# Hansard-T/FHE-Linformer

Measured on AMD Instinct MI355X. Metric: encrypted Linformer-d128 forward ms/sample, lower is better.
Workload: dtype u64

## Files before the change

### fhe-linformer_amd/csrc/context.cpp

```cpp
#include "context.h"
#include <hip/hip_runtime.h>
#include <algorithm>
#include <cstdio>
#include <cstdlib>
#include <cstring>
#include <sys/random.h>
#include <time.h>
#include <cxxabi.h>
#include <dlfcn.h>
#include <execinfo.h>

namespace fhelin {

template <class T>
const T* Context::upload_table(const std::vector<T>& v) {
    void* p = nullptr;
    size_t bytes = std::max<size_t>(v.size() * sizeof(T), 16);
    hip_check(hipMalloc(&p, bytes), "hipMalloc(table)");
    if (!v.empty()) hip_check(hipMemcpy(p, v.data(), v.size() * sizeof(T), hipMemcpyHostToDevice), "hipMemcpy(table)");
    table_allocs.push_back(p);
    return static_cast<const T*>(p);
}
template const u64* Context::upload_table<u64>(const std::vector<u64>&);
template const int* Context::upload_table<int>(const std::vector<int>&);
template const u32* Context::upload_table<u32>(const std::vector<u32>&);
template const double* Context::upload_table<double>(const std::vector<double>&);

static u64 mont_r(u64 m) { return (u64)((((u128)1) << 64) % m); }

static u64 prod_mod(const std::vector<u64>& ms, int skip, u64 t) {
    u64 r = 1 % t;
    for (int i = 0; i < (int)ms.size(); ++i)
        if (i != skip) r = h_mulmod(r, ms[i] % t, t);
    return r;
}

static void resolve_seed(Params& p) {
    if (p.have_seed_bytes) return;
    if (p.seed != 0) {
        std::memset(p.seed_bytes, 0, sizeof p.seed_bytes);
        for (int i = 0; i < 8; ++i) p.seed_bytes[i] = (uint8_t)(p.seed >> (8 * i));
    } else {
        size_t got = 0;
        while (got < sizeof p.seed_bytes) {
            const ssize_t n = getrandom(p.seed_bytes + got, sizeof p.seed_bytes - got, 0);
            if (n <= 0) throw Error(FHELIN_ERR_INTERNAL, "getrandom failed: no entropy for key generation");
            got += (size_t)n;
        }
    }
    p.have_seed_bytes = true;
}

static Params resolve_params(Params p) {
    resolve_seed(p);
    if (p.n_p < 0 && p.n_q >= 1 && p.dnum >= 1 && p.special_bits >= 1) {
        const int a = (p.n_q + p.dnum - 1) / p.dnum;
        const int first = p.first_bits + (std::min(a, p.n_q) - 1) * p.scale_bits;
        const int other = p.n_q > a ? std::min(a, p.n_q - a) * p.scale_bits : 0;
        p.n_p = (std::max(first, other) + p.special_bits - 1) / p.special_bits;
    }
    return p;
}

Context::Context(const Params& p_in) : prm(resolve_params(p_in)) {
    const Params& p = prm;
    if (p.log_n < 12 || p.log_n > 17) throw Error(FHELIN_ERR_ARG, "log_n must be in [12,17]");
    if (p.n_q < 1 || p.n_q > 64 || p.n_p < 0 || p.n_p > 16) throw Error(FHELIN_ERR_ARG, "bad limb counts");
    if (p.dnum < 1) throw Error(FHELIN_ERR_ARG, "dnum must be >= 1");
    if (p.first_bits > 60 || p.scale_bits > 60 || p.special_bits > 60) throw Error(FHELIN_ERR_ARG, "primes must be <= 60 bits");
    if (p.first_bits < 20 || p.scale_bits < 20 || (p.n_p > 0 && p.special_bits < 20)) throw Error(FHELIN_ERR_ARG, "primes must be >= 20 bits");
    if (p.log_slots < 1 || p.log_slots > p.log_n - 1) throw Error(FHELIN_ERR_ARG, "log_slots out of range");
    N = 1 << p.log_n;
    L = p.n_q - 1;
    K = p.n_p;
    alpha = (p.n_q + p.dnum - 1) / p.dnum;
    if (alpha > 16) throw Error(FHELIN_ERR_ARG, "digit size > 16 limbs not supported");
    if ((p.n_q + alpha - 1) / alpha > 16) throw Error(FHELIN_ERR_ARG, "more than 16 key-switching digits not supported");
    try {
        chain = make_prime_chain(p.log_n, p.n_q, p.first_bits, p.scale_bits, p.n_p, p.special_bits);
    } catch (const std::exception& e) {
        throw Error(FHELIN_ERR_ARG, std::string("prime chain: ") + e.what());
    }
    moduli = chain.q;
    moduli.insert(moduli.end(), chain.p.begin(), chain.p.end());
    for (u64 q : moduli)
        if (q >> 60) throw Error(FHELIN_ERR_ARG, "prime chain: a modulus is >= 2^60 (lower scale_bits or first_bits)");
    for (u64 q : moduli) {
        barrett.push_back(h_barrett(q));
        tw.push_back(make_twiddles(q, p.log_n));
    }
    sf_real.assign(p.n_q + 1, 0.0L);
    sf_real[0] = (long double)chain.q[L];
    for (int k = 0; k < L; ++k) sf_real[k + 1] = sf_real[k] * sf_real[k] / (long double)chain.q[L - k];

    pool.fill_word = DevicePool::parse_fill(std::getenv("FHELIN_POOL_FILL"));

    if (p.device < 0) return;

    int ndev = 0;
    if (hipGetDeviceCount(&ndev) != hipSuccess || ndev <= 0)
        throw Error(FHELIN_ERR_NO_DEVICE, "no HIP device visible: the fhe-linformer_amd engine has no CPU fallback");
    if (p.device >= ndev) throw Error(FHELIN_ERR_ARG, "device index out of range");
    hip_check(hipSetDevice(p.device), "hipSetDevice");
    hip_check(hipStreamCreateWithFlags(&stream, hipStreamNonBlocking), "hipStreamCreate");
    main_stream = stream;
    own_stream = true;
    {
        int want = 2;
        if (const char* e = std::getenv("FHELIN_LANES")) want = std::atoi(e);
        n_lanes = std::max(0, std::min(want, DevicePool::MAX_LANES - 1));
        for (int k = 1; k <= n_lanes; ++k) {
            hip_check(hipStreamCreateWithFlags(&lane_stream[k], hipStreamNonBlocking), "hipStreamCreate(lane)");
            hip_check(hipEventCreateWithFlags(&lane_event[k], hipEventDisableTiming), "hipEventCreate(lane)");
        }
        hip_check(hipEventCreateWithFlags(&fork_event, hipEventDisableTiming), "hipEventCreate(fork)");
        pool.lane_stream[0] = main_stream;
        for (int k = 1; k <= n_lanes; ++k) pool.lane_stream[k] = lane_stream[k];
        pool.have_streams = true;
        if (const char* e = std::getenv("FHELIN_ASYNC")) async_lanes = std::atoi(e) != 0;
        if (const char* e = std::getenv("FHELIN_FUSE_MODDOWN")) fuse_moddown = std::atoi(e) != 0;
        if (const char* e = std::getenv("FHELIN_FUSE_FINISH")) fuse_finish = std::atoi(e) != 0;
        if (const char* e = std::getenv("FHELIN_HOST_ENCODE")) host_encode = std::atoi(e) != 0;
        if (const char* e = std::getenv("FHELIN_DEVICE_DECODE")) device_decode = std::atoi(e) != 0;
        if (const char* e = std::getenv("FHELIN_ROT_GATHER")) rot_gather = std::atoi(e) != 0;
        if (const char* e = std::getenv("FHELIN_FUSE_LIFT")) fuse_lift = std::atoi(e) != 0;
        if (const char* e = std::getenv("FHELIN_LDS_DIGITS")) lds_digits = std::atoi(e) != 0;
        if (const char* e = std::getenv("FHELIN_FUSE_ACCP_ROWS")) fuse_accp_rows = std::atoi(e);
        if (const char* e = std::getenv("FHELIN_ACCP_ROWS_MIN_VECS")) accp_rows_min_vecs = std::atoi(e);
        if (const char* e = std::getenv("FHELIN_FUSE_ACCQ_ROWS")) fuse_accq_rows = std::atoi(e);
        if (const char* e = std::getenv("FHELIN_ACCQ_ROWS_MIN_VECS")) accq_rows_min_vecs = std::atoi(e);
        if (const char* e = std::getenv("FHELIN_NTT_TRACE")) trace_small_ntt = std::atoi(e);
        if (const char* e = std::getenv("FHELIN_SCALAR_TRACE")) trace_scalar = std::atoi(e);
        if (const char* e = std::getenv("FHELIN_HOST_WAITS")) trace_waits = std::atoi(e) != 0;
    }
    hip_check(hipEventCreate(&ev_start), "hipEventCreate");
    stage_words = (size_t)2 << p.log_n;
    for (int i = 0; i < STAGE_SLOTS; ++i) {
        hip_check(hipHostMalloc(reinterpret_cast<void**>(&stage_buf[i]), stage_words * sizeof(u64), hipHostMallocDefault), "hipHostMalloc(stage)");
        hip_check(hipEventCreateWithFlags(&stage_ev[i], hipEventDisableTiming), "hipEventCreate(stage)");
    }
    hip_check(hipHostMalloc(reinterpret_cast<void**>(&small_buf), (size_t)SMALL_SLOTS * SMALL_WORDS * sizeof(u64), hipHostMallocDefault), "hipHostMalloc(stage, small)");
    for (int i = 0; i < SMALL_SLOTS; ++i) hip_check(hipEventCreateWithFlags(&small_ev[i], hipEventDisableTiming), "hipEventCreate(stage, small)");
    hip_check(hipEventCreate(&ev_stop), "hipEventCreate");
    has_device = true;

    const int nl = (int)moduli.size();
    {
        std::vector<u64> bar(2 * nl), ninv(8 * nl, 0);
        for (int i = 0; i < nl; ++i) {
            bar[2 * i] = barrett[i].r0;
            bar[2 * i + 1] = barrett[i].r1;
            ninv[8 * i] = tw[i].n_inv;
            ninv[8 * i + 1] = tw[i].n_inv_s;
            ninv[8 * i + 2] = tw[i].w1_n_inv;
            ninv[8 * i + 3] = tw[i].w1_n_inv_s;
            int bits = 0;
            while (bits < 64 && (moduli[i] >> bits)) ++bits;
            if (bits >= 12 && bits <= 60) {
                ninv[8 * i + 4] = (u64)(bits - 10);
                ninv[8 * i + 5] = (u64)((((u128)1) << (bits + 22)) / moduli[i]);
            }
        }
        dt.log_n = p.log_n;
        dt.n_limbs = nl;
        dt.moduli = upload_table(moduli);
        dt.barrett = upload_table(bar);
        {
            std::vector<u64> qi(nl);
            for (int i = 0; i < nl; ++i) {
                u64 x = moduli[i];
                for (int it = 0; it < 6; ++it) x *= 2 - moduli[i] * x;
                qi[i] = x;
            }
            dt.qinv = upload_table(qi);
            std::vector<u64> mr(2 * (size_t)nl);
            for (int i = 0; i < nl; ++i) {
                mr[2 * i] = mont_r(moduli[i]);
                mr[2 * i + 1] = h_shoup(mr[2 * i], moduli[i]);
            }
            dt.mont = upload_table(mr);
        }
        dt.ninv = upload_table(ninv);
        std::vector<u64> f((size_t)nl * 2 * N), g((size_t)nl * 2 * N);
        for (int i = 0; i < nl; ++i) {
            std::memcpy(&f[(size_t)i * 2 * N], tw[i].fwd.data(), sizeof(u64) * 2 * N);
            std::memcpy(&g[(size_t)i * 2 * N], tw[i].inv.data(), sizeof(u64) * 2 * N);
        }
        dt.tw_fwd = upload_table(f);
        dt.tw_inv = upload_table(g);
        const size_t tiles = N >> 12;
        const size_t per_limb = tiles * 15 * 256 * 2;
        for (int dir = 0; dir < 2; ++dir) {
            const std::vector<u64>& src = dir ? g : f;
            std::vector<u64> r((size_t)nl * per_limb);
            for (int i = 0; i < nl; ++i)
                for (size_t T = 0; T < tiles; ++T)
                    for (int kb = 0; kb < 4; ++kb)
                        for (int j = 0; j < (8 >> kb); ++j)
                            for (size_t tau = 0; tau < 256; ++tau) {
                                const size_t idx = (N >> (kb + 1)) + ((((T << 8) | tau)) << (3 - kb)) + j;
                                const size_t s_ = (size_t)(8 >> kb) - 1 + j;
                                const size_t o = (size_t)i * per_limb + ((T * 15 + s_) * 256 + tau) * 2;
                                r[o] = src[(size_t)i * 2 * N + 2 * idx];
                                r[o + 1] = src[(size_t)i * 2 * N + 2 * idx + 1];
                            }
            (dir ? dt.tw_rows_inv : dt.tw_rows_fwd) = upload_table(r);
        }
    }
    {
        std::vector<u64> phatinv(2 * std::max(K, 1)), phatmod((size_t)std::max(K, 1) * (L + 1)), pinv(2 * (L + 1));
        for (int j = 0; j < K; ++j) {
            u64 pj = chain.p[j];
            u64 hat = prod_mod(chain.p, j, pj);
            u64 inv = h_invmod(hat, pj);
            phatinv[2 * j] = inv;
            phatinv[2 * j + 1] = h_shoup(inv, pj);
            for (int t = 0; t <= L; ++t) phatmod[(size_t)j * (L + 1) + t] = pack30(h_mulmod(prod_mod(chain.p, j, chain.q[t]), mont_r(chain.q[t]), chain.q[t]));
        }
        for (int t = 0; t <= L; ++t) {
            u64 qt = chain.q[t];
            u64 pm = prod_mod(chain.p, -1, qt);
            u64 inv = K > 0 ? h_invmod(pm, qt) : 1;
            pinv[2 * t] = inv;
            pinv[2 * t + 1] = h_shoup(inv, qt);
        }
        d_phatinv = upload_table(phatinv);
        d_phatmod = upload_table(phatmod);
        d_pinv = upload_table(pinv);
        std::vector<u64> pmod(2 * (L + 1));
        for (int t = 0; t <= L; ++t) {
            pmod[2 * t] = prod_mod(chain.p, -1, chain.q[t]);
            pmod[2 * t + 1] = h_shoup(pmod[2 * t], chain.q[t]);
        }
        d_pmod = upload_table(pmod);
        std::vector<u64> qlinv((size_t)(L + 1) * (L + 1) * 2, 0), qlmod((size_t)(L + 1) * (L + 1), 0);
        for (int l = 0; l <= L; ++l)
            for (int t = 0; t < l; ++t) {
                u64 qt = chain.q[t];
                u64 r = chain.q[l] % qt;
                u64 inv = h_invmod(r, qt);
                qlmod[(size_t)l * (L + 1) + t] = r;
                qlinv[((size_t)l * (L + 1) + t) * 2] = inv;
                qlinv[((size_t)l * (L + 1) + t) * 2 + 1] = h_shoup(inv, qt);
            }
        d_qlinv = upload_table(qlinv);
        d_qlmod = upload_table(qlmod);
    }
    lvl.resize(L + 2);
    for (int ell = 1; ell <= L + 1; ++ell) {
        LevelTables& lt = lvl[ell];
        lt.ell = ell;
        lt.beta = digits_at(ell);
        const int nt = ell + K;
        std::vector<u64> hatinv(2 * ell), hatmod((size_t)ell * nt, 0), hatmod2((size_t)ell * nt, 0);
        std::vector<int> tab((size_t)lt.beta * nt, -1);
        for (int j = 0; j < lt.beta; ++j) {
            const int lo = j * alpha, hi = std::min((j + 1) * alpha, ell);
            std::vector<u64> dig(chain.q.begin() + lo, chain.q.begin() + hi);
            for (int i = lo; i < hi; ++i) {
                u64 qi = chain.q[i];
                u64 inv = h_invmod(prod_mod(dig, i - lo, qi), qi);
                hatinv[2 * i] = inv;
                hatinv[2 * i + 1] = h_shoup(inv, qi);
                for (int t = 0; t < nt; ++t) {
                    u64 mt = t < ell ? chain.q[t] : chain.p[t - ell];
                    const u64 hr = h_mulmod(prod_mod(dig, i - lo, mt), mont_r(mt), mt);
                    hatmod[(size_t)i * nt + t] = pack30(hr);
                    hatmod2[(size_t)i * nt + t] = pack30(h_mulmod(hr, mont_r(mt), mt));
                }
            }
            for (int t = 0; t < nt; ++t) {
                bool own = t >= lo && t < hi;
                tab[(size_t)j * nt + t] = own ? -1 : (t < ell ? limb_id_q(t) : limb_id_p(t - ell));
            }
        }
        lt.up_hatinv = upload_table(hatinv);
        lt.up_hatmod = upload_table(hatmod);
        lt.up_hatmod_r2 = upload_table(hatmod2);
        lt.ext_limb_tab = upload_table(tab);
        std::vector<int> ktab(nt);
        for (int t = 0; t < nt; ++t) ktab[t] = t < ell ? limb_id_q(t) : limb_id_p(t - ell);
        lt.key_limb_tab = upload_table(ktab);
        if (ell >= 2 && K >= 1) {
// ... 240 lines not shown
```

### fhe-linformer_amd/csrc/context.h

```cpp
#pragma once
#include <cstdint>
#include <map>
#include <memory>
#include <stdexcept>
#include <string>
#include <unordered_map>
#include <vector>
#include <hip/hip_runtime_api.h>
#include "../../include/fhelin.h"
#include "hostmath.h"
#include "pool.h"
#include "kernels_elem.h"

namespace fhelin {

struct Params {
    int log_n = 16;
    int n_q = 24;
    int first_bits = 55;
    int scale_bits = 52;
    int n_p = 6;
    int special_bits = 60;
    int dnum = 4;
    int log_slots = 14;
    int hamming = 192;
    uint64_t seed = 0;
    uint8_t seed_bytes[32] = {};
    bool have_seed_bytes = false;
    int device = 0;
};

struct LevelTables {
    int ell = 0;
    int beta = 0;
    const u64* up_hatinv = nullptr;
    const u64* up_hatmod = nullptr;
    const u64* up_hatmod_r2 = nullptr;
    const int* ext_limb_tab = nullptr;
    const int* key_limb_tab = nullptr;
    const u64* md_hatinv = nullptr;
    const u64* md_hatmod = nullptr;
    const u64* md_minv = nullptr;
    const u64* md_mmod = nullptr;
    const int* mdx_limb_tab = nullptr;
};

struct OpStats {
    u64 limb_ntt = 0;
    u64 keyswitch = 0;
    u64 keyswitch_limbs = 0;
    u64 rescale = 0;
    u64 ct_pt_mult = 0;
    u64 bootstrap = 0;
    u64 encode = 0;
    u64 rescale_limbs = 0;
    u64 ct_pt_limbs = 0;
};

struct Context {
    Params prm;
    OpStats stats;
    int N = 0;
    int L = 0;
    int K = 0;
    int alpha = 0;
    PrimeChain chain;
    std::vector<u64> moduli;
    std::vector<Barrett> barrett;
    std::vector<TwiddleTable> tw;
    std::vector<long double> sf_real;

    bool has_device = false;
    hipStream_t stream = nullptr;
    hipStream_t main_stream = nullptr;
    bool own_stream = false;
    int n_lanes = 0;
    hipStream_t lane_stream[DevicePool::MAX_LANES] = {};
    hipEvent_t lane_event[DevicePool::MAX_LANES] = {};
    hipEvent_t fork_event = nullptr;
    bool async_lanes = true;
    int async_rr = 0;
    u64 lane_seq[DevicePool::MAX_LANES] = {};
    std::vector<std::pair<u64, std::shared_ptr<void>>> lane_hold[DevicePool::MAX_LANES];
    void release_holds(int lane, u64 up_to_seq);
    void fork_lanes();
    void join_lanes();
    DevicePool pool;
    hipStream_t stream_of(int lane) const { return pool.lane_stream[lane]; }
    void select_lane(int lane) {
        stream = stream_of(lane);
        pool.cur_lane = lane;
    }
    void set_main_stream(hipStream_t s) {
        stream = main_stream = pool.lane_stream[0] = s;
        own_stream = false;
    }
    struct LaneScope {
        Context& c;
        hipStream_t was_stream;
        int was_lane;
        LaneScope(Context& ctx, int k) : c(ctx), was_stream(ctx.stream), was_lane(ctx.pool.cur_lane) { c.select_lane(k); }
        ~LaneScope() {
            c.stream = was_stream;
            c.pool.cur_lane = was_lane;
        }
    };
    DeviceTables dt{};
    std::vector<void*> table_allocs;
    hipEvent_t ev_start = nullptr, ev_stop = nullptr;

    static constexpr int STAGE_SLOTS = 64;
    u64* stage_buf[STAGE_SLOTS] = {};
    hipEvent_t stage_ev[STAGE_SLOTS] = {};
    bool stage_used[STAGE_SLOTS] = {};
    int stage_next = 0;
    size_t stage_words = 0;
    static constexpr int SMALL_SLOTS = 256;
    static constexpr size_t SMALL_WORDS = 8192;
    u64* small_buf = nullptr;
    hipEvent_t small_ev[SMALL_SLOTS] = {};
    bool small_used[SMALL_SLOTS] = {};
    int small_next = 0;
    void upload_async(u64* dst, const u64* src, size_t words);

    const u64* d_phatinv = nullptr;
    const u64* d_phatmod = nullptr;
    const u64* d_pinv = nullptr;
    const u64* d_pmod = nullptr;
    const u64* d_qlinv = nullptr;
    const u64* d_qlmod = nullptr;
    std::vector<LevelTables> lvl;
    std::map<u64, const u32*> automorph_maps;

    explicit Context(const Params& p);
    ~Context();
    Context(const Context&) = delete;
    Context& operator=(const Context&) = delete;

    void require_device() const;
    template <class T> T* dalloc(size_t count) { return static_cast<T*>(pool.alloc(count * sizeof(T))); }
    template <class T> Scratch<T> scratch(size_t count) { return Scratch<T>(pool, count); }
    template <class T> const T* upload_table(const std::vector<T>& v);
    int limb_id_q(int i) const { return i; }
    int limb_id_p(int j) const { return L + 1 + j; }
    int digits_at(int ell) const { return (ell + alpha - 1) / alpha; }
    u64 galois_element(long rot_index) const;
    int stride = 1;
    bool stride_explicit = false;
    bool stride_locked = false;
    u64 rot_element(int rot_index) const { return stride == 1 ? galois_element(rot_index) : galois_element((long)stride * rot_index); }
    struct PhysicalScope {
        Context& c;
        int was;
        explicit PhysicalScope(Context& ctx) : c(ctx), was(ctx.stride) { c.stride = 1; }
        ~PhysicalScope() { c.stride = was; }
    };
    const u32* automorph_map(u64 galois);
    const u32* automorph_inverse_of(const u32* map);
    std::map<const u32*, const u32*> automorph_inverse;
    u32 automorph_ginv_of(const u32* map) const;
    std::map<const u32*, u32> automorph_ginv;
    bool fuse_finish = true;
    bool fuse_moddown = false;
    bool host_encode = false;
    bool device_decode = false;
    bool rot_gather = true;
    bool fuse_lift = true;
    int fuse_accp_rows = 1;
    int accp_rows_min_vecs = 0;
    int fuse_accq_rows = 1;
    int accq_rows_min_vecs = 0;
    bool lds_digits = true;
    struct FftDev {
        const u32* rot = nullptr;
        const double* ksi = nullptr;
    };
    std::map<int, FftDev> fft_dev;
    void sync();
    void ntt(const LimbBatch& b, bool inverse, int active = -1) {
        stats.limb_ntt += (u64)(active >= 0 ? active : b.nvec);
        if (trace_small_ntt && b.nvec <= trace_small_ntt) note_small_ntt(b.nvec);
        launch_ntt(dt, b, inverse, stream);
    }
    bool trace_waits = false;
    std::map<std::string, std::pair<u64, u64>> wait_sites;
    void note_wait(const char* site, u64 ns) {
        auto& e = wait_sites[site];
        e.first += 1;
        e.second += ns;
    }
    int trace_small_ntt = 0;
    std::map<std::string, std::pair<u64, u64>> small_ntt_sites;
    void note_small_ntt(int nvec);
    int trace_scalar = 0;
    std::map<std::string, std::pair<u64, u64>> scalar_sites;
    void note_scalar(int nvec);
    void ntt_epilogue(const LimbBatch& b, const NttEpilogue& ep) {
        stats.limb_ntt += (u64)b.nvec;
        if (trace_small_ntt && b.nvec <= trace_small_ntt) note_small_ntt(b.nvec);
        launch_ntt_epilogue(dt, b, ep, stream);
    }
    void ntt_epilogue_product(const LimbBatch& b, const NttEpilogue& ep, const NttProduct& p) {
        stats.limb_ntt += (u64)b.nvec;
        if (trace_small_ntt && b.nvec <= trace_small_ntt) note_small_ntt(b.nvec);
        launch_ntt_epilogue_product(dt, b, ep, p, stream);
    }
};

}
```

### fhe-linformer_amd/csrc/evaluator.cpp

```cpp
#include "evaluator.h"
#include <map>
#include <set>
#include <hip/hip_runtime.h>
#include <cmath>
#include <cstring>

namespace fhelin {

DevBlock::~DevBlock() {
    if (d && ctx) {
        try { ctx->pool.free(d); } catch (...) {}
    }
}
Ciphertext::~Ciphertext() {
    if (async_ev) (void)hipEventDestroy(async_ev);
    if (d && ctx && !block) {
        try { ctx->pool.free(d); } catch (...) {}
    }
}
Encoding::~Encoding() {
    if (ready) (void)hipEventDestroy(ready);
    if (d && ctx) {
        try { ctx->pool.free(d, lanes_ordered); } catch (...) {}
    }
}
EvalKey::~EvalKey() {
    if (d && ctx) {
        try { ctx->pool.free(d); } catch (...) {}
    }
    if (d_perm && ctx) {
        try { ctx->pool.free(d_perm); } catch (...) {}
    }
}

static void launch_ok(const char* what) { hip_check(hipGetLastError(), what); }

namespace {
template <class SameShape, class Emit>
void for_runs(size_t n, SameShape same, Emit emit) {
    size_t lo = 0;
    while (lo < n) {
        size_t hi = lo + 1;
        while (hi < n && hi - lo < (size_t)EwItems::MAX_ITEMS && same(lo, hi)) ++hi;
        emit(lo, hi);
        lo = hi;
    }
}

template <class Same, class Run>
std::vector<CtPtr> for_groups(size_t n, int limit, Same same, Run run) {
    std::vector<CtPtr> out(n);
    std::vector<char> done(n, 0);
    for (size_t first = 0; first < n; ++first) {
        if (done[first]) continue;
        std::vector<size_t> idx{first};
        for (size_t i = first + 1; i < n && (int)idx.size() < limit; ++i)
            if (!done[i] && same(first, i)) idx.push_back(i);
        std::vector<CtPtr> o = run(idx);
        for (size_t k = 0; k < idx.size(); ++k) {
            out[idx[k]] = std::move(o[k]);
            done[idx[k]] = 1;
        }
    }
    return out;
}

std::vector<CtPtr> pick(const std::vector<CtPtr>& v, const std::vector<size_t>& idx) {
    std::vector<CtPtr> o;
    o.reserve(idx.size());
    for (size_t i : idx) o.push_back(v[i]);
    return o;
}
}

CtPtr Evaluator::new_ct(int npoly, int ell, int deg, long double scale, int slots) {
    c_.require_device();
    if (ell < 1 || ell > c_.L + 1 || npoly < 1 || npoly > 3) throw Error(FHELIN_ERR_ARG, "new_ct: bad shape");
    auto ct = std::make_shared<Ciphertext>();
    ct->ctx = &c_;
    ct->npoly = npoly;
    ct->ell = ell;
    ct->deg = deg;
    ct->scale = scale;
    ct->slots = slots;
    ct->d = c_.dalloc<u64>(ct->words());
    c_.stride_locked = true;
    return ct;
}

CtPtr Evaluator::clone(const CtPtr& a) {
    CtPtr o = new_ct(a->npoly, a->ell, a->deg, a->scale, a->slots);
    hip_check(hipMemcpyAsync(o->d, a->d, a->words() * 8, hipMemcpyDeviceToDevice, c_.stream), "clone");
    return o;
}

std::vector<CtPtr> Evaluator::new_ct_batch(int count, int npoly, int ell, int deg, long double scale, int slots) {
    c_.require_device();
    if (count < 1 || ell < 1 || ell > c_.L + 1 + (c_.K > 0 ? 1 : 0) || npoly < 1 || npoly > 3) throw Error(FHELIN_ERR_ARG, "new_ct_batch: bad shape");
    auto blk = std::make_shared<DevBlock>();
    blk->ctx = &c_;
    const size_t words = (size_t)npoly * ell * c_.N;
    blk->d = c_.dalloc<u64>(words * count);
    c_.stride_locked = true;
    std::vector<CtPtr> v;
    for (int i = 0; i < count; ++i) {
        auto ct = std::make_shared<Ciphertext>();
        ct->ctx = &c_;
        ct->npoly = npoly;
        ct->ell = ell;
        ct->deg = deg;
        ct->scale = scale;
        ct->slots = slots;
        ct->block = blk;
        ct->d = blk->d + words * i;
        v.push_back(ct);
    }
    return v;
}

u64* Evaluator::contiguous_base(const std::vector<CtPtr>& v) {
    if (v.empty() || !v[0]->block) return nullptr;
    const size_t words = v[0]->words();
    for (size_t i = 0; i < v.size(); ++i)
        if (v[i]->block != v[0]->block || v[i]->d != v[0]->d + words * i || v[i]->words() != words) return nullptr;
    return v[0]->d;
}

std::vector<CtPtr> Evaluator::make_contiguous(const std::vector<CtPtr>& v, int site) {
    if (v.size() <= 1 || contiguous_base(v)) return v;
    if (site >= 0 && site < 8) gather_copies[site] += v.size();
    std::vector<CtPtr> o = new_ct_batch((int)v.size(), v[0]->npoly, v[0]->ell, v[0]->deg, v[0]->scale, v[0]->slots);
    for (size_t lo = 0; lo < v.size(); lo += EwItems::MAX_ITEMS) {
        EwItems it;
        it.n = (int)std::min<size_t>(EwItems::MAX_ITEMS, v.size() - lo);
        it.vecs = v[0]->npoly * v[0]->ell;
        it.b_vecs = 0;
        for (int i = 0; i < it.n; ++i) {
            if (v[lo + i]->words() != v[0]->words()) throw Error(FHELIN_ERR_INTERNAL, "make_contiguous: operands of different shapes");
            it.out[i] = o[lo + i]->d;
            it.a[i] = v[lo + i]->d;
            it.b[i] = nullptr;
        }
        launch_ew_items(c_.dt, it, 4, v[0]->ell, c_.stream);
    }
    hip_check(hipGetLastError(), "batch gather");
    return o;
}

KeyPtr Evaluator::new_key(int max_ell) {
    c_.require_device();
    if (max_ell < 0 || max_ell > c_.L + 1) throw Error(FHELIN_ERR_ARG, "new_key: max_ell out of range");
    auto k = std::make_shared<EvalKey>();
    k->ctx = &c_;
    k->max_ell = max_ell ? max_ell : c_.L + 1;
    k->digits = c_.digits_at(k->max_ell);
    k->d = c_.dalloc<u64>(k->words());
    if (k->capped()) {
        hip_check(hipMemsetAsync(k->d, 0, k->words() * sizeof(u64), c_.stream), "hipMemsetAsync(capped key)");
    }
    c_.stride_locked = true;
    return k;
}

void Evaluator::bind_key(const EvalKey& key, int ell) {
    if (ell > key.max_ell) {
        std::string who = key.kind == 1 ? "relinearisation key" : key.kind == 3 ? "conjugation key" : "rotation key";
        if (key.kind != 1 && key.has_index) who += " for index " + std::to_string(key.index);
        if (key.kind != 1) who += " (Galois element " + std::to_string((unsigned long long)key.galois) + ")";
        throw Error(FHELIN_ERR_KEY, who + " is capped at " + std::to_string(key.max_ell) + " limbs: a key switch at " + std::to_string(ell) +
                                        " limbs was asked for");
    }
    if (usage_on) {
        int& m = usage[{key.kind, key.galois}];
        m = std::max(m, ell);
    }
}

void Evaluator::bind_rotations(const Rotations& rot, const std::vector<CtPtr>& v, bool rescales_first) {
    for (const CtPtr& x : v)
        for (int r = 0; r < rot.n; ++r) bind_key(*rot.key[r], rescales_first && x->deg >= 2 ? x->ell - 1 : x->ell);
}

void Evaluator::keyswitch(const u64* c_ntt, int ell, const EvalKey& key, u64* out, const u64* add0, const u64* add1,
                          const u32* map, const u64* post) {
    keyswitch_batch(1, c_ntt, 0, ell, key, out, 0, add0, add1, 0, map, post, 0);
}

void Evaluator::keyswitch_batch(int B, const u64* c_ntt, size_t c_stride, int ell, const EvalKey& key, u64* out, size_t out_stride,
                                const u64* add0, const u64* add1, size_t add_stride, const u32* map, const u64* post,
                                size_t post_stride) {
    keyswitch_impl(B, nullptr, c_ntt, c_stride, ell, &key, out, out_stride, add0, add1, add_stride, map, post, post_stride);
}

void Evaluator::keyswitch_rows(const KsRows& rows, const u64* c_ntt, size_t c_stride, int ell, u64* out, size_t out_stride,
                               const u64* add0, size_t add_stride) {
    const int B = (int)rows.keys.size();
    if (B < 1) return;
    if (B > KsShape::MAX_ROWS || rows.maps.size() != rows.keys.size()) throw Error(FHELIN_ERR_ARG, "keyswitch_rows: bad row count");
    keyswitch_impl(B, &rows, c_ntt, c_stride, ell, nullptr, out, out_stride, add0, nullptr, add_stride, nullptr, nullptr, 0);
}

void Evaluator::keyswitch_impl(int B, const KsRows* rows, const u64* c_ntt, size_t c_stride, int ell, const EvalKey* key, u64* out,
                               size_t out_stride, const u64* add0, const u64* add1, size_t add_stride, const u32* map, const u64* post,
                               size_t post_stride) {
    c_.require_device();
    if (c_.K < 1) throw Error(FHELIN_ERR_STATE, "hybrid key switching needs at least one special prime");
    if (B < 1) return;
    if (key) bind_key(*key, ell);
    else
        for (int b = 0; b < B; ++b) bind_key(*rows->keys[b], ell);
    KsShape sh = ks_shape(ell, B, {c_stride, out_stride, add_stride, post_stride});
    const bool shared = rows && rows->shared_input;
    if (rows) {
        sh.per_row = 1;
        sh.shared_input = shared ? 1 : 0;
        for (int b = 0; b < B; ++b) {
            sh.evk_row[b] = rows->keys[b]->d;
            sh.map_row[b] = rows->maps[b];
        }
    }
    KsShape shu = sh;
    shu.batch = shared ? 1 : B;
    c_.stats.keyswitch += (u64)B;
    c_.stats.keyswitch_limbs += (u64)B * ell;
    const bool identity = !map && !rows;
    const bool gather = !identity && !add1 && rot_in_gather();
    const u64* evk = key ? key->d : nullptr;
    if (gather) evk = set_gather(sh, rows ? rows->keys.data() : &key, rows ? rows->maps.data() : &map, add0, add_stride);
    Scratch<u64> ext = modup(shu, c_ntt, !gather);
    KsAcc acc = inner_product(sh, ext, evk, c_ntt, moddown_tail(gather ? KsOutput::Gathered : identity ? KsOutput::Identity : KsOutput::Scattered));
    moddown(acc, gather ? KsOut{out, nullptr, nullptr, post} : KsOut{out, add0, add1, post, map});
    launch_ok("keyswitch");
}


KsShape Evaluator::ks_shape(int ell, int batch, const KsStrides& st) const {
    return KsShape{ell, c_.K, c_.alpha, c_.lvl[ell].beta, c_.L + 1, batch, st.c, st.out, st.add, st.post};
}

Evaluator::KsTail Evaluator::moddown_tail(KsOutput o) const {
    const bool rows = o == KsOutput::Gathered || (o == KsOutput::Identity && (c_.fuse_moddown || c_.fuse_finish)) ||
                      (o == KsOutput::Scattered && c_.fuse_moddown) || (o == KsOutput::MergedSum && c_.fuse_finish && c_.rot_gather);
    return rows ? KsTail::RowPass : KsTail::Finish;
}

const u64* Evaluator::set_gather(KsShape& sh, const EvalKey* const* keys, const u32* const* maps, const u64* c0, size_t c0_stride) {
    const u64* evk = nullptr;
    for (int b = 0; b < (sh.per_row ? (sh.row_mod ? sh.row_mod : sh.batch) : 1); ++b) bind_key(*keys[b], sh.ell);
    sh.gather = 1;
    if (sh.per_row) {
        for (int b = 0; b < (sh.row_mod ? sh.row_mod : sh.batch); ++b) {
            sh.evk_row[b] = permuted(*keys[b], maps[b]);
            sh.ginv_row[b] = c_.automorph_ginv_of(maps[b]);
        }
    } else {
        evk = permuted(*keys[0], maps[0]);
        sh.map_row[0] = maps[0];
        sh.ginv = c_.automorph_ginv_of(maps[0]);
    }
    if (c0) {
        sh.gsrc = c0;
        sh.gsrc_stride = c0_stride;
        sh.gsrc_pmod = c_.d_pmod;
    }
    return evk;
}

Scratch<u64> Evaluator::modup(const KsShape& up, const u64* src, bool times_r2, int group2, size_t group2_stride) {
    const size_t N = c_.N;
    const int n = up.batch, ell = up.ell, nt = ell + c_.K;
    const LevelTables& lt = c_.lvl[ell];
    Scratch<u64> cc = c_.scratch<u64>((size_t)n * ell * N);
    {
        LimbBatch ib{cc, n * ell, nullptr, 0, ell, src};
        if (n > 1 && up.c_stride != (size_t)ell * N) {
            ib.src_group = ell;
            ib.src_group_stride = up.c_stride;
        }
        if (group2 > 0) {
            ib.src_group2 = group2;
            ib.src_group2_stride = group2_stride;
        }
        c_.ntt(ib, true);
    }
    Scratch<u64> ext = c_.scratch<u64>((size_t)n * lt.beta * nt * N);
    launch_modup_conv(c_.dt, up, ext, cc, src, lt.up_hatinv, times_r2 ? lt.up_hatmod_r2 : lt.up_hatmod, c_.stream);
    LimbBatch eb{ext, n * lt.beta * nt, lt.ext_limb_tab, 0, 1};
    eb.tab_len = lt.beta * nt;
    eb.lazy_out = true;
    c_.ntt(eb, false, n * (lt.beta * nt - ell));
    return ext;
}

bool Evaluator::accp_in_rows(const KsShape& sh, KsTail tail) const {
    const int K = c_.K, nvec = sh.batch * 2 * K;
    const bool measured_faster = !sh.n_rot && sh.beta <= 8;
    const bool want = c_.fuse_accp_rows >= 2 || (c_.fuse_accp_rows == 1 && measured_faster);
    return tail != KsTail::EditsAccP && want && !sh.accp_limbs && sh.k == K && nvec >= c_.accp_rows_min_vecs;
}

bool Evaluator::accq_in_rows(const KsShape& sh, KsTail tail) const {
    const bool measured_faster = sh.beta <= 8 && sh.batch * 2 * sh.ell >= c_.accq_rows_min_vecs;
    const bool want = c_.fuse_accq_rows >= 2 || (c_.fuse_accq_rows == 1 && measured_faster);
    return tail == KsTail::RowPass && !sh.n_rot && want;
}

Evaluator::KsAcc Evaluator::accumulators(const KsShape& sh, KsTail tail) {
    const size_t pairs = (size_t)sh.batch * 2 * c_.N;
    return KsAcc{sh, tail, c_.scratch<u64>(pairs * sh.ell), c_.scratch<u64>(pairs * (sh.accp_limbs ? sh.accp_limbs : sh.k)), {}};
}

Evaluator::KsAcc Evaluator::inner_product(const KsShape& shape, const u64* ext, const u64* evk, const u64* c_ntt, KsTail tail) {
    const int K = c_.K, nvec = shape.batch * 2 * K;
    KsAcc acc{shape, tail, {}, {}, {}};
    KsShape& sh = acc.sh;
    sh.accp_rows = accp_in_rows(sh, tail) ? 1 : 0;
    sh.accq_rows = sh.accp_rows && accq_in_rows(sh, tail) ? 1 : 0;
    if (!sh.accq_rows) acc.accQ = c_.scratch<u64>((size_t)sh.batch * 2 * sh.ell * c_.N);
    acc.accP = c_.scratch<u64>((size_t)nvec * c_.N);
    if (sh.n_rot) launch_ks_inner_multi(c_.dt, sh, acc.accQ, acc.accP, ext, c_ntt, c_.stream);
    else if (!sh.accq_rows) launch_ks_inner(c_.dt, sh, acc.accQ, acc.accP, ext, evk, c_ntt, c_.stream);
    if (!sh.accp_rows) return acc;
    acc.qprod = NttProduct{sh, ext, evk, sh.n_rot ? 1 : 0, c_ntt};
    c_.stats.limb_ntt += (u64)nvec;
    launch_ntt_rows_product(c_.dt, LimbBatch{acc.accP, nvec, nullptr, c_.L + 1, K}, acc.qprod, c_.stream);
    return acc;
}

void Evaluator::accp_inverse(KsAcc& acc) {
    const LimbBatch b{acc.accP, acc.sh.batch * 2 * c_.K, nullptr, c_.L + 1, c_.K};
    if (acc.sh.accp_rows) launch_ntt_cols_inverse(c_.dt, b, c_.stream);
    else c_.ntt(b, true);
}

static void made_for(bool ok, const char* tail) {
    if (!ok) throw Error(FHELIN_ERR_INTERNAL, std::string(tail) + ": the accumulator was made for another tail");
}

Scratch<u64> Evaluator::moddown_conv(KsAcc& acc) {
    const KsShape& sh = acc.sh;
    made_for(acc.tail == KsTail::RowPass || acc.tail == KsTail::Finish, "moddown");
    if (acc.tail == KsTail::RowPass && sh.gsrc && !sh.gsrc_pmod) throw Error(FHELIN_ERR_INTERNAL, "moddown: the row pass cannot gather");
    accp_inverse(acc);
    Scratch<u64> conv = c_.scratch<u64>((size_t)sh.batch * 2 * sh.ell * c_.N);
    launch_moddown_conv(c_.dt, sh, conv, acc.accP, c_.d_phatinv, c_.d_phatmod, c_.stream);
    if (acc.tail != KsTail::RowPass) c_.ntt(LimbBatch{conv, sh.batch * 2 * sh.ell, nullptr, 0, sh.ell}, false);
    return conv;
}

void Evaluator::moddown(KsAcc& acc, const KsOut& o) {
    Scratch<u64> conv = moddown_conv(acc);
    if (acc.tail == KsTail::RowPass) moddown_rows(acc, conv, o);
    else launch_moddown_finish(c_.dt, acc.sh, o.out, acc.accQ, conv, c_.d_pinv, o.add0, o.add1, o.map, o.post, c_.stream);
}

void Evaluator::moddown_rows(const KsAcc& acc, u64* conv, const KsOut& o) {
    const KsShape& sh = acc.sh;
    const int B = sh.batch, ell = sh.ell;
    const LimbBatch cb{conv, B * 2 * ell, nullptr, 0, ell};
    NttEpilogue ep;
    ep.acc = acc.accQ;
    ep.acc_poly_stride = (size_t)ell * c_.N;
    ep.out = o.out;
    ep.out_stride = sh.out_stride;
    ep.w = c_.d_pinv;
    ep.ell = ell;
    ep.add0 = o.add0;
    ep.add1 = o.add1;
    ep.add_stride = sh.add_stride;
    ep.post = o.post;
    ep.post_stride = sh.post_stride;
    if (sh.gather) {
    } else if (sh.per_row) {
        ep.per_row = 1;
        for (int b = 0; b < B; ++b) ep.invmap_row[b] = c_.automorph_inverse_of(sh.map_row[b]);
    } else if (o.map) {
        ep.invmap = c_.automorph_inverse_of(o.map);
    }
    if (sh.accq_rows) c_.ntt_epilogue_product(cb, ep, acc.qprod);
    else c_.ntt_epilogue(cb, ep);
}

void Evaluator::moddown_rescale(KsAcc& acc, u64* out) {
    const KsShape& sh = acc.sh;
    const size_t N = c_.N;
    const int B = sh.batch, ell = sh.ell;
    const LevelTables& lt = c_.lvl[ell];
    made_for(acc.tail == KsTail::Rescale || acc.tail == KsTail::EditsAccP, "moddown_rescale");
    accp_inverse(acc);
    Scratch<u64> top = c_.scratch<u64>((size_t)B * 2 * N);
    {
        LimbBatch tb{top, B * 2, nullptr, ell - 1, 1, acc.accQ + (size_t)(ell - 1) * N};
        tb.src_group = 1;
        tb.src_group_stride = (size_t)ell * N;
        c_.ntt(tb, true);
    }
    Scratch<u64> conv = c_.scratch<u64>((size_t)B * 2 * (ell - 1) * N);
    launch_moddown_rescale_conv(c_.dt, sh, conv, acc.accP, top, lt.md_hatinv, lt.md_hatmod, lt.md_mmod, c_.stream);
    moddown_rescale_finish(acc, out, conv, lt.md_minv);
}

void Evaluator::moddown_rescale_exact(KsAcc& acc, u64* out, u32 f2) {
    const KsShape& sh = acc.sh;
    const int B = sh.batch, ell = sh.ell, K = c_.K;
    const LevelTables& lt = c_.lvl[ell];
    made_for(acc.tail == KsTail::Exact, "moddown_rescale_exact");
    {
        LimbBatch ib{acc.accP, B * 2 * (K + 1), lt.mdx_limb_tab, 0, 1};
        ib.tab_len = K + 1;
        c_.ntt(ib, true);
    }
    Scratch<u64> conv = c_.scratch<u64>((size_t)B * 2 * (ell - 1) * c_.N);
    launch_moddown_rescale_exact_conv(c_.dt, sh, f2, conv, acc.accP, c_.d_phatinv, c_.d_phatmod, c_.d_pinv, c_.d_pmod,
                                      c_.d_qlmod + (size_t)(ell - 1) * (c_.L + 1), c_.stream);
    moddown_rescale_finish(acc, out, conv, lt.md_minv);
}

void Evaluator::moddown_rescale_finish(const KsAcc& acc, u64* out, u64* conv, const u64* minv) {
    const KsShape& sh = acc.sh;
    const int e1 = sh.ell - 1;
    const LimbBatch cb{conv, sh.batch * 2 * e1, nullptr, 0, e1};
    if (c_.fuse_finish) {
        NttEpilogue ep;
        ep.acc = acc.accQ;
        ep.acc_poly_stride = (size_t)sh.ell * c_.N;
        ep.out = out;
        ep.out_stride = sh.out_stride;
        ep.w = minv;
        ep.ell = e1;
        c_.ntt_epilogue(cb, ep);
        return;
    }
    c_.ntt(cb, false);
    launch_moddown_rescale_finish(c_.dt, sh, out, acc.accQ, conv, minv, c_.stream);
}

Evaluator::Rotations Evaluator::rotations(const int* indices, int n) {
    Rotations rot;
    rot.n = n;
    for (int r = 0; r < n; ++r) {
        const RotKey k = rotation_key(indices[r]);
        rot.key[r] = k.key.get();
        rot.map[r] = k.map;
        if (k.g % (u64)(c_.N / 256) != 1) rot.tiles_in_place = false;
    }
    return rot;
}

void Evaluator::set_rotations(KsShape& sh, const Rotations& rot, bool shared_digits, const u64* const* keys) {
    for (int r = 0; r < rot.n; ++r) bind_key(*rot.key[r], sh.ell);
    sh.n_rot = rot.n;
    for (int r = 0; r < rot.n; ++r) {
        sh.map_rot[r] = rot.map[r];
        sh.evk_rot[r] = keys ? keys[r] : permuted(*rot.key[r], rot.map[r]);
    }
    if (shared_digits) sh.lds_digits = c_.lds_digits && rot.tiles_in_place ? 1 : 0;
}

void Evaluator::rotation_sum(KsShape& sh, const u64* ext, const u64* base, size_t c0_stride, const KsOut& o) {
    const KsTail tail = moddown_tail(KsOutput::MergedSum);
    sh.gsrc = base;
    sh.gsrc_stride = c0_stride;
    if (tail == KsTail::RowPass) sh.gsrc_pmod = c_.d_pmod;
    KsAcc acc = inner_product(sh, ext, nullptr, base + (size_t)sh.ell * c_.N, tail);
    moddown(acc, o);
}

Scratch<u64> Evaluator::debug_ks_accp(const u64* ext, int ell, int batch, const int* indices, int n_rot) {
    const size_t pn = (size_t)ell * c_.N;
    if (ell < 1 || ell > c_.L + 1 || batch < 1 || n_rot < 0 || n_rot > (int)KsShape::MAX_ROT) throw Error(FHELIN_ERR_ARG, "debug_ks_accp: bad shape");
    if (!n_rot && !relin_key) throw Error(FHELIN_ERR_KEY, "debug_ks_accp: no relinearisation key");
    if (!n_rot) bind_key(*relin_key, ell);
    KsShape sh = ks_shape(ell, batch, {pn});
    Scratch<u64> own = c_.scratch<u64>((size_t)batch * pn);
    hip_check(hipMemsetAsync(own, 0, (size_t)batch * pn * sizeof(u64), c_.stream), "hipMemsetAsync(debug_ks_accp)");
    if (n_rot) set_rotations(sh, rotations(indices, n_rot), true, nullptr);
    KsAcc acc = inner_product(sh, ext, n_rot ? nullptr : relin_key->d, own, KsTail::Finish);
    accp_inverse(acc);
    launch_ok("debug_ks_accp");
    return std::move(acc.accP);
}

void Evaluator::debug_ks_accq(const u64* ext, const u64* own, u64* conv, int ell, int batch, int index, u64* out) {
    const size_t pn = (size_t)ell * c_.N;
    if (ell < 1 || ell > c_.L + 1 || batch < 1) throw Error(FHELIN_ERR_ARG, "debug_ks_accq: bad shape");
    if (!index && !relin_key) throw Error(FHELIN_ERR_KEY, "debug_ks_accq: no relinearisation key");
    if (!index) bind_key(*relin_key, ell);
    KsShape sh = ks_shape(ell, batch, {pn, 2 * pn});
    const u64* evk = index ? nullptr : relin_key->d;
    if (index) {
        const RotKey k = rotation_key(index);
        const EvalKey* key = k.key.get();
        evk = set_gather(sh, &key, &k.map);
    }
    KsAcc acc = inner_product(sh, ext, evk, own, KsTail::RowPass);
    moddown_rows(acc, conv, KsOut{out});
    launch_ok("debug_ks_accq");
}

int Evaluator::slot_count(int slots) const { return slots > 0 ? slots : (1 << c_.prm.log_slots); }

Evaluator::RotKey Evaluator::rotation_key(int index) {
    const u64 g = c_.rot_element(index);
    auto it = rot_keys.find(g);
    if (it == rot_keys.end()) throw Error(FHELIN_ERR_KEY, "no rotation key for index " + std::to_string(index) + " (EvalRotateKeyGen list)");
    return RotKey{it->second, c_.automorph_map(g), g};
}

bool Evaluator::have_rotation_keys(const std::vector<int>& indices, int slots) const {
    const int ns = slot_count(slots);
    for (int r : indices) {
        if (r % ns == 0) return false;
        if (!rot_keys.count(c_.rot_element(r))) return false;
    }
    return !indices.empty();
}

const u64* Evaluator::permuted(const EvalKey& key, const u32* map) {
    if (key.d_perm) return key.d_perm;
    const int nvec = key.digits * 2 * (c_.L + 1 + c_.K);
    key.d_perm = c_.dalloc<u64>(key.words());
    launch_automorph_pack30(c_.dt, key.d_perm, key.d, map, nvec, c_.stream);
    launch_ok("key permutation");
    hip_check(hipStreamSynchronize(c_.stream), "key permutation sync");
    return key.d_perm;
}

std::vector<CtPtr> Evaluator::rotate_sum_batch(const std::vector<CtPtr>& vin, const std::vector<int>& indices) {
    if (vin.empty()) return {};
    const int R = (int)indices.size();
    if (R < 1 || R > KsShape::MAX_ROT) throw Error(FHELIN_ERR_ARG, "rotate_sum_batch: 1..7 rotations");
    if (!have_rotation_keys(indices, vin[0]->slots)) throw Error(FHELIN_ERR_KEY, "rotate_sum_batch: missing rotation key");
    if (c_.K < 1) throw Error(FHELIN_ERR_STATE, "hybrid key switching needs at least one special prime");
    const Rotations rot = rotations(indices.data(), R);
    bind_rotations(rot, vin);
    const size_t N = c_.N;
    return for_groups(vin.size(), batch_limit, [&](size_t f, size_t i) { return same_shape(*vin[f], *vin[i]); },
                      [&](const std::vector<size_t>& idx) {
        if (vin[idx[0]]->npoly != 2) throw Error(FHELIN_ERR_STATE, "rotate: ciphertext must have 2 components");
        const std::vector<CtPtr> chunk = make_contiguous(pick(vin, idx), 0);
        const int B = (int)chunk.size(), ell = chunk[0]->ell;
        const size_t pn = (size_t)ell * N, ctw = 2 * pn;
        std::vector<CtPtr> o = new_ct_batch(B, 2, ell, chunk[0]->deg, chunk[0]->scale, chunk[0]->slots);
        const u64* base = chunk[0]->d;
        KsShape sh = ks_shape(ell, B, {ctw, ctw, pn, ctw});
        set_rotations(sh, rot, true);
        int steps = 0;
        while ((1 << steps) < R + 1) ++steps;
        c_.stats.keyswitch += (u64)B * steps;
        c_.stats.keyswitch_limbs += (u64)B * steps * ell;
        {
            Scratch<u64> ext = modup(sh, base + pn, false);
            rotation_sum(sh, ext, base, ctw, KsOut{o[0]->d, nullptr, nullptr, base});
            launch_ok("rotate_sum_batch");
        }
        for (int b = 0; b < B; ++b) o[b]->scale = vin[idx[b]]->scale;
        return o;
    });
}

Evaluator::FoldedKey Evaluator::folded_key(const PtPtr& p, int index, long double scale) {
    const RotKey rk = rotation_key(index);
    for (size_t i = 0; i < folded_keys.size(); ++i) {
        const FoldedKey& f = folded_keys[i];
        if (f.pt.get() == p.get() && f.key.get() == rk.key.get() && f.index == index && f.scale == scale) {
            FoldedKey hit = f;
            if (i + 1 != folded_keys.size()) {
                folded_keys.erase(folded_keys.begin() + i);
                folded_keys.push_back(hit);
            }
            return hit;
        }
    }
    FoldedKey f;
    f.pt = p;
    f.key = rk.key;
    f.index = index;
    f.scale = scale;
    const int nl = c_.L + 1 + c_.K;
    f.enc = p->at(nl, scale);
    f.d = std::make_shared<DevBlock>();
    f.d->ctx = &c_;
    f.d->d = c_.dalloc<u64>(f.key->words());
    launch_fold_key(c_.dt, f.d->d, f.key->d, rk.map, f.enc->d, f.key->digits * 2 * nl, c_.stream);
    launch_ok("fold_key");
// ... 1010 lines not shown
}

void Evaluator::rescale_degree2(std::vector<CtPtr>& a, std::vector<CtPtr>* b, const char* two_components) {
    std::vector<CtPtr> need;
    std::map<const Ciphertext*, size_t> slot;
    for (const auto* side : {&a, b})
        for (size_t i = 0; side && i < side->size(); ++i) {
            const CtPtr& c = (*side)[i];
            if (two_components && c->npoly != 2) throw Error(FHELIN_ERR_STATE, two_components);
            if (c->deg >= 2 && !slot.count(c.get())) {
                slot[c.get()] = need.size();
                need.push_back(c);
            }
        }
    if (need.empty()) return;
    const std::vector<CtPtr> r = rescale_batch(need);
    for (auto* side : {&a, b})
        for (size_t i = 0; side && i < side->size(); ++i) {
            CtPtr& c = (*side)[i];
            if (c->deg >= 2) c = r[slot[c.get()]];
        }
}

std::vector<CtPtr> Evaluator::tensor_products(const std::vector<CtPtr>& x, const std::vector<CtPtr>& y, const std::vector<size_t>& idx) {
    const int B = (int)idx.size(), ell = x[idx[0]]->ell;
    std::vector<CtPtr> d = new_ct_batch(B, 3, ell, 2, 0, x[idx[0]]->slots);
    for (int k0 = 0; k0 < B; k0 += EwItems::MAX_ITEMS) {
        EwItems it;
        it.n = std::min(B - k0, (int)EwItems::MAX_ITEMS);
        for (int k = 0; k < it.n; ++k) {
            it.out[k] = d[k0 + k]->d;
            it.a[k] = x[idx[k0 + k]]->d;
            it.b[k] = y[idx[k0 + k]]->d;
        }
        launch_tensor_items(c_.dt, it, ell, c_.stream);
    }
    return d;
}

void Evaluator::product_operands(const std::vector<CtPtr>& a, const std::vector<CtPtr>& b, std::vector<CtPtr>& x, std::vector<CtPtr>& y) {
    std::vector<CtPtr> ra = a, rb = b;
    rescale_degree2(ra, &rb, "mult: operands must have 2 components");
    match_batch(ra, rb, x, y);
}

std::vector<CtPtr> Evaluator::mult_batch(const std::vector<CtPtr>& a, const std::vector<CtPtr>& b) {
    if (a.size() != b.size()) throw Error(FHELIN_ERR_ARG, "mult_batch: operand count mismatch");
    if (!relin_key) throw Error(FHELIN_ERR_KEY, "no relinearisation key (EvalMultKeyGen not called)");
    std::vector<CtPtr> x, y;
    product_operands(a, b, x, y);
    for (const CtPtr& xi : x) bind_key(*relin_key, xi->ell);
    std::vector<CtPtr> out = for_groups(a.size(), batch_limit, [&](size_t f, size_t i) { return x[i]->ell == x[f]->ell; },
                                        [&](const std::vector<size_t>& idx) {
        const int B = (int)idx.size(), ell = x[idx[0]]->ell;
        const size_t pn = (size_t)ell * c_.N;
        const std::vector<CtPtr> d = tensor_products(x, y, idx);
        std::vector<CtPtr> o = new_ct_batch(B, 2, ell, 2, 0, x[idx[0]]->slots);
        keyswitch_batch(B, d[0]->d + 2 * pn, 3 * pn, ell, *relin_key, o[0]->d, 2 * pn, d[0]->d, d[0]->d + pn, 3 * pn, nullptr, nullptr, 0);
        for (int k = 0; k < B; ++k) {
            const size_t i = idx[k];
            o[k]->deg = x[i]->deg + y[i]->deg;
            o[k]->scale = x[i]->scale * y[i]->scale;
        }
        return o;
    });
    launch_ok("mult_batch");
    return out;
}

std::vector<CtPtr> Evaluator::mult_affine_rescale_batch(const std::vector<CtPtr>& a, const std::vector<CtPtr>& b, int f, double cadd,
                                                        const std::vector<CtPtr>& sub) {
    if (a.size() != b.size() || (!sub.empty() && sub.size() != a.size())) throw Error(FHELIN_ERR_ARG, "mult_affine_rescale_batch: operand count mismatch");
    if (f != 1 && f != 2) throw Error(FHELIN_ERR_ARG, "mult_affine_rescale_batch: factor 1 or 2");
    if (!relin_key) throw Error(FHELIN_ERR_KEY, "no relinearisation key (EvalMultKeyGen not called)");
    if (c_.K < 1 || c_.K + 1 > 16) throw Error(FHELIN_ERR_STATE, "mult_affine_rescale_batch: 1..15 special primes");
    std::vector<CtPtr> ra = a, rb = b, x(a.size()), y(a.size());
    rescale_degree2(ra, &rb, "mult: operands must have 2 components");
    for (size_t i = 0; i < a.size(); ++i) match(ra[i], rb[i], x[i], y[i]);
    for (const CtPtr& xi : x) bind_key(*relin_key, xi->ell);
    const size_t N = c_.N;
    const int K = c_.K, L1 = c_.L + 1;
    hipStream_t s = c_.stream;
    auto product_scale = [&](size_t i) { return x[i]->scale * y[i]->scale; };
    return for_groups(a.size(), batch_limit,
                      [&](size_t f0, size_t i) { return x[i]->ell == x[f0]->ell && fabsl(product_scale(i) / product_scale(f0) - 1.0L) < 1e-12L; },
                      [&](const std::vector<size_t>& idx) {
        const size_t first = idx[0];
        const int B = (int)idx.size(), ell = x[first]->ell;
        if (ell < 2) throw Error(FHELIN_ERR_STATE, "mult_affine_rescale_batch: no limb left to drop");
        const size_t pn = (size_t)ell * N;
        const long double sc = product_scale(first);
        const std::vector<CtPtr> d = tensor_products(x, y, idx);
        std::vector<CtPtr> sadj;
        if (!sub.empty()) {
            for (int k = 0; k < B; ++k) sadj.push_back(adjust(sub[idx[k]], ell, 2, sc));
            sadj = make_contiguous(sadj, 7);
        }
        ScalarSet cst;
        if (cadd != 0.0) real_to_scalars(c_, (long double)cadd * sc, ell, cst);
        KsShape sh = ks_shape(ell, B, {3 * pn, (size_t)2 * (ell - 1) * N, pn});
        c_.stats.keyswitch += (u64)B;
        c_.stats.keyswitch_limbs += (u64)B * ell;
        c_.stats.rescale += (u64)B;
        c_.stats.rescale_limbs += (u64)B * ell;
        const u64* c_ntt = d[0]->d + 2 * pn;
        std::vector<CtPtr> o = new_ct_batch(B, 2, ell - 1, 1, 0, x[first]->slots);
        {
            Scratch<u64> ext = modup(sh, c_ntt, true);
            KsAcc acc = inner_product(sh, ext, relin_key->d, c_ntt, f == 2 ? KsTail::EditsAccP : KsTail::Rescale);
            launch_affine_acc(c_.dt, sh, acc.accQ, d[0]->d, sadj.empty() ? nullptr : sadj[0]->d, cst, cadd != 0.0 ? 1 : 0, f, c_.d_pmod, s);
            if (f == 2) launch_ew_add(c_.dt, acc.accP, acc.accP, acc.accP, B * 2 * K, B * 2 * K, L1, K, s);
            moddown_rescale(acc, o[0]->d);
            launch_ok("mult_affine_rescale_batch");
        }
        for (int k = 0; k < B; ++k) o[k]->scale = product_scale(idx[k]) / (long double)c_.chain.q[ell - 1];
        return o;
    });
}

std::vector<CtPtr> Evaluator::mult_affine_unmerged(const std::vector<CtPtr>& a, const std::vector<CtPtr>& b, const std::vector<AffineSpec>& spec) {
    std::vector<CtPtr> t = mult_batch(a, b);
    const size_t n = t.size();
    {
        std::vector<size_t> pos;
        std::vector<CtPtr> sel;
        for (size_t i = 0; i < n; ++i)
            if (spec[i].f == 2) {
                pos.push_back(i);
                sel.push_back(t[i]);
            }
        if (!sel.empty()) {
            const std::vector<CtPtr> r = add_batch(sel, sel);
            for (size_t j = 0; j < pos.size(); ++j) t[pos[j]] = r[j];
        }
    }
    for (size_t i = 0; i < n; ++i)
        if (spec[i].cadd != 0.0) t[i] = add_real(t[i], spec[i].cadd);
    for (const bool neg : {true, false}) {
        std::vector<size_t> pos;
        std::vector<CtPtr> sel, ad;
        for (size_t i = 0; i < n; ++i)
            if (spec[i].addend && spec[i].negate == neg) {
                pos.push_back(i);
                sel.push_back(t[i]);
                ad.push_back(spec[i].addend);
            }
        if (sel.empty()) continue;
        const std::vector<CtPtr> r = neg ? sub_batch(sel, ad) : add_batch(sel, ad);
        for (size_t j = 0; j < pos.size(); ++j) t[pos[j]] = r[j];
    }
    return rescale_batch(t);
}

std::vector<CtPtr> Evaluator::mult_affine_batch(const std::vector<CtPtr>& a, const std::vector<CtPtr>& b, const std::vector<AffineSpec>& spec) {
    if (a.size() != b.size() || spec.size() != a.size()) throw Error(FHELIN_ERR_ARG, "mult_affine_batch: operand count mismatch");
    if (!relin_key) throw Error(FHELIN_ERR_KEY, "no relinearisation key (EvalMultKeyGen not called)");
    for (const AffineSpec& sp : spec) {
        if (sp.f != 1 && sp.f != 2) throw Error(FHELIN_ERR_ARG, "mult_affine_batch: factor 1 or 2");
        if (sp.addend && sp.addend->npoly != 2) throw Error(FHELIN_ERR_STATE, "add: component count mismatch");
    }
    if (!exact_products_on()) return mult_affine_unmerged(a, b, spec);
    const size_t n = a.size();
    std::vector<CtPtr> x, y;
    product_operands(a, b, x, y);
    for (const CtPtr& xi : x) bind_key(*relin_key, xi->ell);
    for (size_t i = 0; i < n; ++i)
        if (x[i]->ell < 2 || (spec[i].addend && spec[i].addend->ell < x[i]->ell)) return mult_affine_unmerged(x, y, spec);
    const size_t N = c_.N;
    const int K = c_.K;
    hipStream_t s = c_.stream;
    static_assert(AffineItems::MAX_ITEMS <= EwItems::MAX_ITEMS, "the tensor products of a group are one launch");
    return for_groups(n, std::min(batch_limit, (int)AffineItems::MAX_ITEMS), [&](size_t f, size_t i) { return x[i]->ell == x[f]->ell; },
                      [&](const std::vector<size_t>& idx) {
        const size_t first = idx[0];
        const int B = (int)idx.size(), ell = x[first]->ell;
        const size_t pn = (size_t)ell * N;
        const std::vector<CtPtr> d = tensor_products(x, y, idx);
        AffineItems items;
        std::vector<CtPtr> adj(B);
        std::map<std::pair<const Ciphertext*, long double>, CtPtr> adjusted;
        std::vector<u64> cst((size_t)B * ell, 0);
        for (int k = 0; k < B; ++k) {
            const size_t i = idx[k];
            const AffineSpec& sp = spec[i];
            const long double sc = x[i]->scale * y[i]->scale;
            if (sp.f == 2) items.f2 |= 1u << k;
            if (sp.addend) {
                const CtPtr& ad = sp.addend;
                const std::pair<const Ciphertext*, long double> key{ad.get(), sc};
                auto hit = ad->deg == 1 ? adjusted.find(key) : adjusted.end();
                if (hit != adjusted.end()) {
                    adj[k] = hit->second;
                } else {
                    adj[k] = ad->ell == ell && ad->deg == 2 ? ad : adjust(ad, ell, 2, sc);
                    if (ad->deg == 1) adjusted[key] = adj[k];
                }
                items.add[k] = adj[k]->d;
                if (sp.negate) items.neg |= 1u << k;
            }
            if (sp.cadd != 0.0) {
                ScalarSet one;
                real_to_scalars(c_, (long double)sp.cadd * sc, ell, one);
                for (int l = 0; l < ell; ++l) cst[(size_t)k * ell + l] = one.v[2 * l];
                items.cst |= 1u << k;
            }
        }
        Scratch<u64> dcst = c_.scratch<u64>(cst.size());
        if (items.cst) c_.upload_async(dcst, cst.data(), cst.size());
        KsShape sh = ks_shape(ell, B, {3 * pn, (size_t)2 * (ell - 1) * N, pn});
        sh.accp_limbs = K + 1;
        c_.stats.keyswitch += (u64)B;
        c_.stats.keyswitch_limbs += (u64)B * ell;
        c_.stats.rescale += (u64)B;
        c_.stats.rescale_limbs += (u64)B * ell;
        const u64* c_ntt = d[0]->d + 2 * pn;
        std::vector<CtPtr> o = new_ct_batch(B, 2, ell - 1, 1, 0, x[first]->slots);
        {
            Scratch<u64> ext = modup(sh, c_ntt, true);
            KsAcc acc = accumulators(sh, KsTail::Exact);
            launch_ks_inner(c_.dt, sh, acc.accQ, acc.accP, ext, relin_key->d, c_ntt, s);
            launch_affine_acc_items(c_.dt, sh, items, acc.accQ, acc.accP, d[0]->d, dcst, c_.d_pmod, s);
            moddown_rescale_exact(acc, o[0]->d, items.f2);
            launch_ok("mult_affine_batch");
        }
        for (int k = 0; k < B; ++k) o[k]->scale = x[idx[k]]->scale * y[idx[k]]->scale / (long double)c_.chain.q[ell - 1];
        return o;
    });
}

std::vector<CtPtr> Evaluator::add_plain_batch(const std::vector<CtPtr>& v, const PtPtr& p) {
    std::vector<CtPtr> out(v.size());
    for_runs(v.size(), [&](size_t a, size_t b) { return v[a]->npoly == v[b]->npoly && v[a]->ell == v[b]->ell; },
             [&](size_t lo, size_t hi) {
                 const CtPtr& f = v[lo];
                 std::vector<CtPtr> o = new_ct_batch((int)(hi - lo), f->npoly, f->ell, f->deg, f->scale, f->slots);
                 EwItems it;
                 it.n = (int)(hi - lo);
                 it.vecs = f->npoly * f->ell;
                 it.b_vecs = f->ell;
                 for (size_t i = lo; i < hi; ++i) {
                     auto enc = p->at(v[i]->ell, v[i]->scale);
                     o[i - lo]->deg = v[i]->deg;
                     o[i - lo]->scale = v[i]->scale;
                     it.out[i - lo] = o[i - lo]->d;
                     it.a[i - lo] = v[i]->d;
                     it.b[i - lo] = enc->d;
                     out[i] = o[i - lo];
                 }
                 launch_ew_items(c_.dt, it, 3, f->ell, c_.stream);
             });
    launch_ok("add_plain_batch");
    return out;
}

CtPtr Evaluator::rotate_add(const CtPtr& a, int index) {
    if (index % slot_count(a) == 0) return add(a, a);
    const RotKey k = rotation_key(index);
    return raw_rotate(a, k.g, *k.key, true, k.map);
}

CtPtr Evaluator::raw_mult_relin(const CtPtr& a, const CtPtr& b, const EvalKey& key) {
    if (a->npoly != 2 || b->npoly != 2 || a->ell != b->ell) throw Error(FHELIN_ERR_STATE, "mult: operands must be 2-component, same level");
    const int ell = a->ell;
    const size_t pn = (size_t)ell * c_.N;
    Scratch<u64> d = c_.scratch<u64>(3 * pn);
    launch_tensor(c_.dt, d, a->d, b->d, ell, c_.stream);
    CtPtr o = new_ct(2, ell, a->deg + b->deg, a->scale * b->scale, a->slots);
    keyswitch(d + 2 * pn, ell, key, o->d, d, d + pn, nullptr);
    return o;
}

CtPtr Evaluator::raw_modraise(const CtPtr& a, int new_ell) {
    if (a->ell != 1) throw Error(FHELIN_ERR_STATE, "modraise: the input must have exactly one limb (q0)");
    if (new_ell < 1 || new_ell > c_.L + 1) throw Error(FHELIN_ERR_ARG, "modraise: bad target limb count");
    const size_t N = c_.N;
    const int P = a->npoly;
    hipStream_t s = c_.stream;
    Scratch<u64> coef = c_.scratch<u64>((size_t)P * N);
    LimbBatch ib{coef, P, nullptr, 0, 1, a->d};
    c_.ntt(ib, true);
    CtPtr up = new_ct(P, new_ell, a->deg, a->scale, a->slots);
    launch_modraise(c_.dt, up->d, coef, P, 0, new_ell, s);
    c_.ntt(LimbBatch{up->d, P * new_ell, nullptr, 0, new_ell}, false);
    launch_ok("modraise");
    return up;
}

std::vector<CtPtr> Evaluator::raw_modraise_batch(const std::vector<CtPtr>& vin, int new_ell) {
    if (vin.size() <= 1) {
        std::vector<CtPtr> out;
        for (const CtPtr& a : vin) out.push_back(raw_modraise(a, new_ell));
        return out;
    }
    for (const CtPtr& a : vin)
        if (a->ell != 1 || a->npoly != vin[0]->npoly) throw Error(FHELIN_ERR_STATE, "modraise: the inputs must have exactly one limb (q0) and one shape");
    if (new_ell < 1 || new_ell > c_.L + 1) throw Error(FHELIN_ERR_ARG, "modraise: bad target limb count");
    std::vector<CtPtr> in = make_contiguous(vin, 7);
    const size_t N = c_.N;
    const int B = (int)in.size(), P = in[0]->npoly * B;
    hipStream_t s = c_.stream;
    Scratch<u64> coef = c_.scratch<u64>((size_t)P * N);
    c_.ntt(LimbBatch{coef, P, nullptr, 0, 1, in[0]->d}, true);
    std::vector<CtPtr> up = new_ct_batch(B, in[0]->npoly, new_ell, 1, 0, in[0]->slots);
    launch_modraise(c_.dt, up[0]->d, coef, P, 0, new_ell, s);
    c_.ntt(LimbBatch{up[0]->d, P * new_ell, nullptr, 0, new_ell}, false);
    launch_ok("modraise_batch");
    coef.reset();
    for (int b = 0; b < B; ++b) {
        up[b]->deg = vin[b]->deg;
        up[b]->scale = vin[b]->scale;
        up[b]->slots = vin[b]->slots;
    }
    return up;
}

CtPtr Evaluator::rescale(const CtPtr& a) {
    CtPtr o = raw_rescale(a);
    o->scale = a->scale / (long double)c_.chain.q[a->ell - 1];
    o->deg = a->deg > 1 ? a->deg - 1 : 1;
    return o;
}

CtPtr Evaluator::level_reduce(const CtPtr& a, int new_ell) {
    if (new_ell == a->ell) return a;
    if (new_ell < 1 || new_ell > a->ell) throw Error(FHELIN_ERR_ARG, "level_reduce: bad target");
    CtPtr o = new_ct(a->npoly, new_ell, a->deg, a->scale, a->slots);
    const size_t N = c_.N;
    hip_check(hipMemcpy2DAsync(o->d, (size_t)new_ell * N * 8, a->d, (size_t)a->ell * N * 8, (size_t)new_ell * N * 8, a->npoly,
                               hipMemcpyDeviceToDevice, c_.stream), "level_reduce");
    return o;
}

CtPtr Evaluator::mult_int(const CtPtr& a, u64 k, bool raise_deg, long double new_scale, int keep_ell) {
    const int ell = keep_ell > 0 ? std::min(keep_ell, a->ell) : a->ell;
    ScalarSet sc;
    for (int i = 0; i < ell; ++i) {
        u64 q = c_.chain.q[i];
        u64 v = k % q;
        sc.v[2 * i] = v;
        sc.v[2 * i + 1] = h_shoup(v, q);
    }
    CtPtr o = new_ct(a->npoly, ell, raise_deg ? a->deg + 1 : a->deg, new_scale, a->slots);
    if (c_.trace_scalar) c_.note_scalar(a->npoly * ell);
    launch_ew_scalar(c_.dt, o->d, a->d, sc, a->npoly * ell, 0, ell, c_.stream, ell < a->ell ? a->ell : 0);
    launch_ok("mult_int");
    return o;
}

std::vector<CtPtr> Evaluator::adjust_deg1_batch(const std::vector<CtPtr>& v, int ell, long double scale) {
    return adjust_deg1_batch(v, ell, std::vector<long double>(v.size(), scale));
}

std::vector<CtPtr> Evaluator::adjust_deg1_batch(const std::vector<CtPtr>& v, int ell, const std::vector<long double>& scales) {
    if (scales.size() != v.size()) throw Error(FHELIN_ERR_ARG, "adjust_deg1_batch: one target scale per ciphertext");
    std::vector<CtPtr> out(v.size()), pending, src;
    std::vector<size_t> pos;
    for (size_t i = 0; i < v.size(); ++i) {
        CtPtr cur = v[i];
        if (cur->ell < ell) throw Error(FHELIN_ERR_STATE, "adjust: cannot raise a ciphertext to a lower level");
        if (cur->deg == 2) cur = rescale(cur);
        if (cur->ell == ell) {
            out[i] = cur;
            continue;
        }
        src.push_back(cur);
        pos.push_back(i);
    }
    if (!src.empty()) {
        const long double qdrop = (long double)c_.chain.q[ell];
        const int lim = ell + 1;
        pending.assign(src.size(), CtPtr());
        std::map<int, std::vector<size_t>> by_npoly;
        for (size_t j = 0; j < src.size(); ++j) by_npoly[src[j]->npoly].push_back(j);
        for (const auto& g : by_npoly) {
// ... 239 lines not shown
```

### fhe-linformer_amd/csrc/evaluator.h

```cpp
#pragma once
#include <cmath>
#include <map>
#include <memory>
#include <vector>
#include "context.h"
#include "kernels_elem.h"

namespace fhelin {

struct DevBlock {
    Context* ctx = nullptr;
    u64* d = nullptr;
    ~DevBlock();
};

struct Ciphertext {
    Context* ctx = nullptr;
    u64* d = nullptr;
    std::shared_ptr<DevBlock> block;
    int npoly = 2;
    int ell = 0;
    int deg = 1;
    long double scale = 0;
    int slots = 0;
    bool async_pending = false;
    int async_lane = 0;
    u64 async_seq = 0;
    hipEvent_t async_ev = nullptr;
    bool seeded = false;
    u64 nonce = 0;
    uint8_t seed[32] = {};
    std::vector<int> wrap_pos;
    int wrap_total = 0;
    bool wrapped() const { return !wrap_pos.empty(); }
    ~Ciphertext();
    int level() const { return ctx->L + 1 - ell; }
    size_t words() const { return (size_t)npoly * ell * ctx->N; }
};
typedef std::shared_ptr<Ciphertext> CtPtr;

struct Encoding {
    Context* ctx = nullptr;
    u64* d = nullptr;
    int ell = 0;
    int ell_q = 0;
    long double scale = 0;
    hipEvent_t ready = nullptr;
    int made_lane = 0;
    unsigned lanes_ordered = 0;
    ~Encoding();
};

struct Plaintext {
    Context* ctx = nullptr;
    std::vector<double> values;
    std::vector<double> imag;
    int slots = 0;
    int stride = 1;
    int level = 0;
    double max_abs = 0.0;
    static constexpr size_t MAX_ENCODINGS = 16;
    std::vector<std::shared_ptr<Encoding>> cache;
    std::shared_ptr<Encoding> at(int ell, long double scale, int ell_q = 0);
    std::shared_ptr<Encoding> at_sliced(int ell_q, long double scale);
    size_t sliced_bytes() const {
        size_t b = 0;
        for (const auto& e : cache)
            if (e->ell_q > 0) b += (size_t)e->ell * ctx->N * 8;
        return b;
    }
    std::shared_ptr<Plaintext> shared;
    static constexpr size_t MAX_SHARED_ENCODINGS = 64;
    bool fixed = false;
};
typedef std::shared_ptr<Plaintext> PtPtr;

struct EvalKey {
    Context* ctx = nullptr;
    u64* d = nullptr;
    mutable u64* d_perm = nullptr;
    int digits = 0;
    bool seeded = false;
    int max_ell = 0;
    int kind = 0;
    u64 galois = 0;
    bool has_index = false;
    int index = 0;
    bool capped() const { return max_ell < ctx->L + 1; }
    ~EvalKey();
    size_t words() const { return (size_t)digits * 2 * (ctx->L + 1 + ctx->K) * ctx->N; }
};
typedef std::shared_ptr<EvalKey> KeyPtr;

inline bool same_scale(const Ciphertext& a, const Ciphertext& b) { return fabsl(b.scale / a.scale - 1.0L) < 1e-9L; }
inline bool same_shape(const Ciphertext& a, const Ciphertext& b) {
    return a.npoly == 2 && b.npoly == 2 && a.ell == b.ell && a.deg == b.deg && same_scale(a, b);
}

void real_to_scalars(const Context& c, long double v, int ell, ScalarSet& sc);

class Evaluator {
public:
    explicit Evaluator(Context& c) : c_(c) {}
    Context& ctx() { return c_; }

    CtPtr new_ct(int npoly, int ell, int deg, long double scale, int slots);
    std::vector<CtPtr> new_ct_batch(int count, int npoly, int ell, int deg, long double scale, int slots);
    static u64* contiguous_base(const std::vector<CtPtr>& v);
    std::vector<CtPtr> make_contiguous(const std::vector<CtPtr>& v, int site = -1);
    u64 gather_copies[8] = {};
    bool dot_groups = true;
    bool cheb_leaf_at_product = true;
    bool cheb_leaf_classes = true;
    bool cheb_rounds = true;
    bool adjust_items = true;
    int batch_limit = 32;
    CtPtr clone(const CtPtr& a);
    KeyPtr new_key(int max_ell = 0);

    void bind_key(const EvalKey& key, int ell);
    bool usage_on = false;
    std::map<std::pair<int, u64>, int> usage;

    std::map<u64, KeyPtr> rot_keys;
    KeyPtr relin_key;
    KeyPtr conj_key;

    void keyswitch(const u64* c_ntt, int ell, const EvalKey& key, u64* out, const u64* add0, const u64* add1, const u32* map,
                   const u64* post = nullptr);
    void keyswitch_batch(int batch, const u64* c_ntt, size_t c_stride, int ell, const EvalKey& key, u64* out, size_t out_stride,
                         const u64* add0, const u64* add1, size_t add_stride, const u32* map, const u64* post, size_t post_stride);
    struct KsRows {
        std::vector<const EvalKey*> keys;
        std::vector<const u32*> maps;
        bool shared_input = false;
    };
    void keyswitch_rows(const KsRows& rows, const u64* c_ntt, size_t c_stride, int ell, u64* out, size_t out_stride, const u64* add0,
                        size_t add_stride);
    std::vector<CtPtr> rotate_sum_batch(const std::vector<CtPtr>& v, const std::vector<int>& indices);
    bool have_rotation_keys(const std::vector<int>& indices, int slots) const;
    const u64* permuted(const EvalKey& key, const u32* map);
    CtPtr rotate_each_sum(const std::vector<CtPtr>& v, const std::vector<int>& indices);
    std::vector<CtPtr> rotate_each_sum_rows(const std::vector<std::vector<CtPtr>>& rows, const std::vector<int>& indices);
    std::vector<CtPtr> hoisted_dot_rows(const std::vector<CtPtr>& xs, const std::vector<PtPtr>& pts, const std::vector<int>& indices,
                                        bool rescale_out = false);
    static int lt_split_cost(const std::vector<int>& idx, int n1);
    std::vector<CtPtr> linear_transform_rows(const std::vector<CtPtr>& xs, const std::vector<std::vector<PtPtr>>& pts,
                                             const std::vector<int>& baby, const std::vector<int>& giant, bool rescale_out = false,
                                             long double pt_scale = 0);
    bool merged_products = false;
    bool merged_rescale = true;
    bool double_hoist = true;
    struct FoldedKey {
        PtPtr pt;
        KeyPtr key;
        int index = 0;
        long double scale = 0;
        std::shared_ptr<Encoding> enc;
        std::shared_ptr<DevBlock> d;
    };
    std::vector<FoldedKey> folded_keys;
    static constexpr size_t MAX_FOLDED = 12;
    FoldedKey folded_key(const PtPtr& p, int index, long double scale);
    std::vector<CtPtr> rotate_many(const CtPtr& a, const std::vector<int>& indices);
    std::vector<std::vector<CtPtr>> rotate_many_batch(const std::vector<CtPtr>& xs, const std::vector<int>& indices);
    Scratch<u64> debug_ks_accp(const u64* ext, int ell, int batch, const int* indices, int n_rot);
    void debug_ks_accq(const u64* ext, const u64* own, u64* conv, int ell, int batch, int index, u64* out);
    std::vector<CtPtr> rotate_galois_batch(const std::vector<CtPtr>& v, u64 galois, const EvalKey& key, bool accumulate);
    std::vector<CtPtr> conjugate_batch(const std::vector<CtPtr>& v);
    std::vector<CtPtr> raw_modraise_batch(const std::vector<CtPtr>& v, int new_ell);
    std::vector<CtPtr> rotate_each(const std::vector<CtPtr>& v, const std::vector<int>& indices);
    std::vector<CtPtr> rotate_add_batch(const std::vector<CtPtr>& v, int index);
    std::vector<CtPtr> rotate_batch(const std::vector<CtPtr>& v, int index);
    std::vector<CtPtr> rotate_batch_impl(const std::vector<CtPtr>& v, int index, bool accumulate);
    std::vector<CtPtr> mult_plain_batch(const std::vector<CtPtr>& v, const PtPtr& p);
    std::vector<CtPtr> mult_plain_each(const std::vector<CtPtr>& v, const std::vector<PtPtr>& p);
    bool dot_plain_groups(const std::vector<CtPtr>& cts, const std::vector<std::vector<PtPtr>>& pts, long double pt_scale,
                          const std::vector<CtPtr>& dest);
    bool dot_plain_cyclic(const std::vector<CtPtr>& cts, const std::vector<PtPtr>& pts, const std::vector<CtPtr>& dest);
    bool dot_plain_window(const std::vector<CtPtr>& cur, const std::vector<CtPtr>& prev, const std::vector<PtPtr>& pts,
                          const std::vector<CtPtr>& dest, bool accumulate);
    bool dot_plain_groups_batch(const std::vector<std::vector<CtPtr>>& cts, const std::vector<std::vector<PtPtr>>& pts, long double pt_scale,
                                const std::vector<std::vector<CtPtr>>& dest);
    CtPtr dot_plain(const std::vector<CtPtr>& v, const std::vector<PtPtr>& p, long double pt_scale = 0,
                    const CtPtr& dest = CtPtr());
    std::vector<CtPtr> add_batch(const std::vector<CtPtr>& a, const std::vector<CtPtr>& b);
    std::vector<CtPtr> add_plain_batch(const std::vector<CtPtr>& v, const PtPtr& p);
    std::vector<CtPtr> sub_batch(const std::vector<CtPtr>& a, const std::vector<CtPtr>& b);
    std::vector<CtPtr> mult_batch(const std::vector<CtPtr>& a, const std::vector<CtPtr>& b);
    std::vector<CtPtr> mult_affine_rescale_batch(const std::vector<CtPtr>& a, const std::vector<CtPtr>& b, int f, double cadd,
                                                 const std::vector<CtPtr>& sub);
    struct AffineSpec {
        int f = 1;
        double cadd = 0;
        CtPtr addend;
        bool negate = false;
    };
    bool exact_products = true;
    bool exact_products_on() const { return exact_products && c_.K >= 1 && c_.K + 1 <= 16; }
    std::vector<CtPtr> mult_affine_batch(const std::vector<CtPtr>& a, const std::vector<CtPtr>& b, const std::vector<AffineSpec>& spec);
    std::vector<CtPtr> eval_chebyshev_many(const std::vector<CtPtr>& xs, const std::vector<double>& coeffs, double a, double b);
    std::vector<CtPtr> rescale_batch(const std::vector<CtPtr>& v);

    CtPtr add(const CtPtr& a, const CtPtr& b);
    CtPtr sub(const CtPtr& a, const CtPtr& b);
    CtPtr negate(const CtPtr& a);
    CtPtr add_plain(const CtPtr& a, const PtPtr& p);
    CtPtr mult_plain(const CtPtr& a, const PtPtr& p);
    CtPtr mult(const CtPtr& a, const CtPtr& b);
    CtPtr mult_no_relin(const CtPtr& a, const CtPtr& b);
    CtPtr relinearize(const CtPtr& a);
    CtPtr mult_int(const CtPtr& a, u64 k, bool raise_deg, long double new_scale, int keep_ell = 0);
    std::vector<CtPtr> adjust_deg1_batch(const std::vector<CtPtr>& v, int ell, long double scale);
    std::vector<CtPtr> adjust_deg1_batch(const std::vector<CtPtr>& v, int ell, const std::vector<long double>& scales);
    std::vector<CtPtr> scaled_diff_batch(const std::vector<CtPtr>& u, const std::vector<CtPtr>& w, const std::vector<u128>& a,
                                         const std::vector<u128>& c, bool raise_deg, const std::vector<long double>& scales);
    CtPtr mult_real(const CtPtr& a, double c);
    CtPtr add_real(const CtPtr& a, double c);
    CtPtr lincomb(const std::vector<CtPtr>& terms, const std::vector<double>& coef, double c0);
    CtPtr lincomb_at(const std::vector<CtPtr>& terms, const std::vector<double>& coef, double c0, long double want_scale, int keep_ell);
    CtPtr rotate(const CtPtr& a, int index);
    CtPtr conjugate(const CtPtr& a);
    CtPtr eval_poly(const CtPtr& x, const std::vector<double>& coeffs);
    CtPtr eval_chebyshev(const CtPtr& x, const std::vector<double>& coeffs, double a, double b);
    CtPtr mult_many(const std::vector<CtPtr>& v);
    std::vector<CtPtr> eval_poly_many(const std::vector<CtPtr>& xs, const std::vector<double>& coeffs);
    std::vector<CtPtr> mult_many_rows(const std::vector<std::vector<CtPtr>>& vs);
    CtPtr rescale(const CtPtr& a);
    CtPtr level_reduce(const CtPtr& a, int new_ell);
    CtPtr adjust(const CtPtr& a, int ell, int deg, long double scale);

    CtPtr raw_rescale(const CtPtr& a);
    void lift_and_ntt(u64* lifted, const u64* last, int P, int ell, const NttEpilogue* ep = nullptr, const u64* qlm_row = nullptr);
    void rescale_finish(u64* out, const u64* c, const u64* last, int P, int ell, const u64* qlinv_row = nullptr, const u64* qlm_row = nullptr);
    CtPtr raw_rotate(const CtPtr& a, u64 galois, const EvalKey& key, bool accumulate = false, const u32* map = nullptr);
    CtPtr rotate_add(const CtPtr& a, int index);
    CtPtr raw_mult_relin(const CtPtr& a, const CtPtr& b, const EvalKey& key);
    CtPtr raw_modraise(const CtPtr& a, int new_ell);

private:
    Context& c_;
    void keyswitch_impl(int batch, const KsRows* rows, const u64* c_ntt, size_t c_stride, int ell, const EvalKey* key, u64* out,
                        size_t out_stride, const u64* add0, const u64* add1, size_t add_stride, const u32* map, const u64* post,
                        size_t post_stride);
    struct KsStrides { size_t c = 0, out = 0, add = 0, post = 0; };
    KsShape ks_shape(int ell, int batch, const KsStrides& st) const;
    enum class KsTail {
        RowPass,
        Finish,
        Rescale,
        Exact,
        EditsAccP,
    };
    struct KsAcc {
        KsShape sh;
        KsTail tail;
        Scratch<u64> accQ;
        Scratch<u64> accP;
        NttProduct qprod;
    };
    struct KsOut {
        u64* out = nullptr;
        const u64 *add0 = nullptr, *add1 = nullptr, *post = nullptr;
        const u32* map = nullptr;
    };
    enum class KsOutput { Identity, Gathered, Scattered, MergedSum };
    KsTail moddown_tail(KsOutput o) const;
    const u64* set_gather(KsShape& sh, const EvalKey* const* keys, const u32* const* maps, const u64* c0 = nullptr, size_t c0_stride = 0);
    Scratch<u64> modup(const KsShape& up, const u64* src, bool times_r2, int group2 = 0, size_t group2_stride = 0);
    KsAcc inner_product(const KsShape& sh, const u64* ext, const u64* evk, const u64* c_ntt, KsTail tail);
    KsAcc accumulators(const KsShape& sh, KsTail tail);
    bool accp_in_rows(const KsShape& sh, KsTail tail) const;
    bool accq_in_rows(const KsShape& sh, KsTail tail) const;
    void accp_inverse(KsAcc& acc);
    Scratch<u64> moddown_conv(KsAcc& acc);
    void moddown(KsAcc& acc, const KsOut& o);
    void moddown_rows(const KsAcc& acc, u64* conv, const KsOut& o);
    void moddown_rescale(KsAcc& acc, u64* out);
    void moddown_rescale_exact(KsAcc& acc, u64* out, u32 f2);
    int slot_count(int slots) const;
    int slot_count(const CtPtr& a) const { return slot_count(a->slots); }
    struct RotKey {
        const KeyPtr& key;
        const u32* map;
        u64 g;
    };
    RotKey rotation_key(int index);
    struct Rotations {
        int n = 0;
        const EvalKey* key[KsShape::MAX_ROT] = {};
        const u32* map[KsShape::MAX_ROT] = {};
        bool tiles_in_place = true;
    };
    Rotations rotations(const int* indices, int n);
    void bind_rotations(const Rotations& rot, const std::vector<CtPtr>& v, bool rescales_first = false);
    void set_rotations(KsShape& sh, const Rotations& rot, bool shared_digits, const u64* const* keys = nullptr);
    void rotation_sum(KsShape& sh, const u64* ext, const u64* base, size_t c0_stride, const KsOut& o);
    void rescale_degree2(std::vector<CtPtr>& a, std::vector<CtPtr>* b = nullptr, const char* two_components = nullptr);
    std::vector<CtPtr> tensor_products(const std::vector<CtPtr>& x, const std::vector<CtPtr>& y, const std::vector<size_t>& idx);
    void product_operands(const std::vector<CtPtr>& a, const std::vector<CtPtr>& b, std::vector<CtPtr>& x, std::vector<CtPtr>& y);
    std::vector<CtPtr> mult_affine_unmerged(const std::vector<CtPtr>& a, const std::vector<CtPtr>& b, const std::vector<AffineSpec>& spec);
    bool rot_in_gather() const { return c_.fuse_finish && c_.rot_gather && !c_.fuse_moddown; }
    void moddown_rescale_finish(const KsAcc& acc, u64* out, u64* conv, const u64* minv);
    typedef std::vector<CtPtr> CtRow;
    CtRow cheb_recurse(const std::vector<double>& c, const std::vector<CtRow>& T, const std::map<int, CtRow>& G, int baby);
    std::vector<CtPtr> add_sub_batch(const std::vector<CtPtr>& a, const std::vector<CtPtr>& b, int op);
    void match(const CtPtr& a, const CtPtr& b, CtPtr& ao, CtPtr& bo);
    void match_batch(const std::vector<CtPtr>& a, const std::vector<CtPtr>& b, std::vector<CtPtr>& x, std::vector<CtPtr>& y);
};

}
```

### fhe-linformer_amd/csrc/kernels_elem.h

```cpp
#pragma once
#include "kernels.h"

namespace fhelin {

struct ScalarSet {
    u64 v[128];
};

void launch_ew_mul(const DeviceTables& t, u64* out, const u64* a, const u64* b, int nvec, int b_mod, int limb_first, int limb_count, hipStream_t s);
void launch_ew_add(const DeviceTables& t, u64* out, const u64* a, const u64* b, int nvec, int b_mod, int limb_first, int limb_count, hipStream_t s);
void launch_ew_sub(const DeviceTables& t, u64* out, const u64* a, const u64* b, int nvec, int b_mod, int limb_first, int limb_count, hipStream_t s);
void launch_ew_muladd(const DeviceTables& t, u64* out, const u64* acc, const u64* a, const u64* b, int nvec, int b_mod, int limb_first,
                      int limb_count, hipStream_t s);
void launch_ew_neg(const DeviceTables& t, u64* out, const u64* a, int nvec, int limb_first, int limb_count, hipStream_t s);
void launch_ew_scalar(const DeviceTables& t, u64* out, const u64* a, const ScalarSet& sc, int nvec, int limb_first, int limb_count, hipStream_t s,
                      int in_limbs = 0);
void launch_ew_addscalar(const DeviceTables& t, u64* out, const u64* a, const ScalarSet& sc, int nvec, int limb_first, int limb_count, hipStream_t s,
                         int add_vecs = -1);
struct LinComb {
    static constexpr int MAX_TERMS = 32;
    int n = 0;
    int vecs = 0;
    const u64* a[MAX_TERMS];
};
void launch_ew_lincomb(const DeviceTables& t, u64* out, const LinComb& lc, const u64* scal, int ell, hipStream_t s, int in_limbs = 0);
void launch_tensor(const DeviceTables& t, u64* d, const u64* a, const u64* b, int ell, hipStream_t s);
struct EwItems;
void launch_tensor_items(const DeviceTables& t, const EwItems& it, int ell, hipStream_t s);
void launch_automorph(const DeviceTables& t, u64* out, const u64* in, const u32* map, int nvec, hipStream_t s);
void launch_automorph_pack30(const DeviceTables& t, u64* out, const u64* in, const u32* map, int nvec, hipStream_t s);
struct WrapMaskRow {
    const u64* src;
    u64* dst;
    const u64* mask;
    const u32* map;
    int32_t ell;
    int32_t src_ell;
};
static_assert(sizeof(WrapMaskRow) == 40, "WrapMaskRow is 40 bytes");
void launch_wrap_mask(const DeviceTables& t, const WrapMaskRow* rows, int n_rows, int max_ell, hipStream_t s);
void launch_rescale_lift(const DeviceTables& t, u64* lifted, const u64* last, int npoly, int ell, const u64* qlmod_row, hipStream_t s);
void launch_rescale_finish(const DeviceTables& t, u64* out, const u64* c, const u64* lifted, int npoly, int ell, const u64* qlinv_row,
                           hipStream_t s);
void launch_modraise(const DeviceTables& t, u64* out, const u64* src, int npoly, int src_limb, int nl, hipStream_t s);
void launch_reduce_i128(const DeviceTables& t, u64* out, const u64* coeffs, int limb_first, int nlimbs, hipStream_t s);

struct EwItems {
    static constexpr int MAX_ITEMS = 32;
    int n = 0;
    int vecs = 0;
    int b_vecs = 0;
    u64* out[MAX_ITEMS];
    const u64* a[MAX_ITEMS];
    const u64* b[MAX_ITEMS];
};
void launch_ew_items(const DeviceTables& t, const EwItems& it, int op, int limb_count, hipStream_t s);
struct EwScaledDiff {
    static constexpr int MAX_ITEMS = 32;
    int n = 0;
    int vecs = 0;
    int ell = 0;
    u64* out[MAX_ITEMS];
    const u64* u[MAX_ITEMS];
    const u64* w[MAX_ITEMS];
};
void launch_ew_scaled_diff(const DeviceTables& t, const EwScaledDiff& d, const u64* consts, hipStream_t s);
struct EwScalarItems {
    static constexpr int MAX_ITEMS = EwItems::MAX_ITEMS;
    int n = 0;
    int npoly = 0;
    int ell = 0;
    int in_limbs[MAX_ITEMS];
    const u64* a[MAX_ITEMS];
};
void launch_ew_scalar_items(const DeviceTables& t, const EwScalarItems& d, u64* out, const u64* consts, hipStream_t s);
struct EwPairPack {
    static constexpr int MAX_PAIRS = 32;
    int n = 0;
    int ell_a[MAX_PAIRS];
    int ell_b[MAX_PAIRS];
    const u64* a[MAX_PAIRS];
    const u64* b[MAX_PAIRS];
};
void launch_ew_pair_pack(const DeviceTables& t, const EwPairPack& d, u64* out, const u64* mono_i, const u64* consts, hipStream_t s);
struct EwPairSplit {
    static constexpr int MAX_PAIRS = 32;
    int n = 0;
    int ell = 0;
    const u64* w[MAX_PAIRS];
    const u64* wc[MAX_PAIRS];
    u64* a[MAX_PAIRS];
    u64* b[MAX_PAIRS];
};
void launch_ew_pair_split(const DeviceTables& t, const EwPairSplit& d, const u64* mono_i, hipStream_t s);
void launch_ew_dot(const DeviceTables& t, u64* out, const EwItems& it, int limb_count, hipStream_t s);
struct EwDotGroups {
    static constexpr int MAX_A = 16, MAX_G = 8;
    int na = 0, ng = 0, ell = 0;
    const u64* a[MAX_A];
    const u64* p[MAX_G][MAX_A];
    u64* out[MAX_G];
    int nbatch = 1;
    size_t a_stride[MAX_A] = {};
    size_t out_stride[MAX_G] = {};
    u32 pmask[MAX_G] = {};
};
void launch_ew_dot_groups(const DeviceTables& t, const EwDotGroups& d, hipStream_t s);
struct EwCyclic {
    static constexpr int PERIOD = 32;
    int n = 0, ell = 0;
    const u64* a[PERIOD];
    const u64* m[PERIOD];
    u64* out[PERIOD];
};
void launch_ew_cyclic_dot(const DeviceTables& t, const EwCyclic& d, hipStream_t s);
struct EwWindow {
    static constexpr int W = 32;
    int ell = 0, accumulate = 0;
    u32 cur_mask = 0, prev_mask = 0;
    const u64* cur[W];
    const u64* prev[W];
    const u64* m[W];
    u64* out[W];
};
void launch_ew_window_dot(const DeviceTables& t, const EwWindow& d, hipStream_t s);

struct KsShape {
    int ell;
    int k;
    int alpha;
    int beta;
    int L1;
    int batch = 1;
    size_t c_stride = 0;
    size_t out_stride = 0;
    size_t add_stride = 0;
    size_t post_stride = 0;
    static constexpr int MAX_ROWS = 16;
    int per_row = 0;
    int shared_input = 0;
    int row_mod = 0;
    const u64* evk_row[MAX_ROWS] = {};
    const u32* map_row[MAX_ROWS] = {};
    static constexpr int MAX_ROT = 7;
    int n_rot = 0;
    const u64* evk_rot[MAX_ROT] = {};
    const u32* map_rot[MAX_ROT] = {};
    size_t rot_ext_stride = 0;
    size_t rot_input_stride = 0;
    int lds_digits = 0;
    size_t ext_batch_stride = 0;
    const u64* gsrc = nullptr;
    size_t gsrc_stride = 0;
    const u64* gsrc_pmod = nullptr;
    int gather = 0;
    u32 ginv = 0;
    u32 ginv_row[MAX_ROWS] = {};
    int tch = 16;
    int accp_limbs = 0;
    int accp_rows = 0;
    int accq_rows = 0;
};
struct NttProduct {
    KsShape sh;
    const u64* ext = nullptr;
    const u64* evk = nullptr;
    int multi = 0;
    const u64* c_ntt = nullptr;
};
void launch_ntt_rows_product(const DeviceTables& t, const LimbBatch& b, const NttProduct& p, hipStream_t s);
void launch_ntt_epilogue_product(const DeviceTables& t, const LimbBatch& b, const NttEpilogue& ep, const NttProduct& p, hipStream_t s);
void launch_ntt_cols_inverse(const DeviceTables& t, const LimbBatch& b, hipStream_t s);
void launch_modup_conv(const DeviceTables& t, const KsShape& sh, u64* ext, const u64* cc, const u64* c_ntt, const u64* hatinv,
                       const u64* hatmod, hipStream_t s);
void launch_ks_inner(const DeviceTables& t, const KsShape& sh, u64* accQ, u64* accP, const u64* ext, const u64* evk, const u64* c_ntt,
                     hipStream_t s);
void launch_ks_inner_multi(const DeviceTables& t, const KsShape& sh, u64* accQ, u64* accP, const u64* ext, const u64* c_ntt,
                           hipStream_t s);
void launch_fold_key(const DeviceTables& t, u64* out, const u64* key, const u32* map, const u64* V, int nvec, hipStream_t s);
struct HoistAdd {
    int n_rot = 0;
    const u64* v[KsShape::MAX_ROT + 1] = {};
    const u32* map[KsShape::MAX_ROT] = {};
    u64* acc = nullptr;
    const u64* pmod = nullptr;
};
void launch_hoist_addends(const DeviceTables& t, const KsShape& sh, const HoistAdd& h, u64* pre, const u64* ct, hipStream_t s);
struct LtStep {
    static constexpr int MAX_G = 4;
    const u64* key;
    const u32* map;
    const u64* v[MAX_G];
    u32 mask;
    u32 pad;
};
struct LtDot {
    static constexpr int MAX_STEPS = 32;
    const LtStep* steps = nullptr;
    int n_steps = 0;
    int n_groups = 0;
    int g0 = 0, groups = 0;
    const u64* pmod = nullptr;
    int dense_v = 0;
};
void launch_ks_inner_dot(const DeviceTables& t, const KsShape& sh, const LtDot& ld, u64* accQ, u64* accP, const u64* ext, const u64* c0,
                         const u64* c1, hipStream_t s);
void launch_moddown_conv(const DeviceTables& t, const KsShape& sh, u64* conv, const u64* accP, const u64* phatinv, const u64* phatmod,
                         hipStream_t s);
void launch_affine_acc(const DeviceTables& t, const KsShape& sh, u64* accQ, const u64* d, const u64* sub, const ScalarSet& cst, int has_cst, int f,
                       const u64* pmod, hipStream_t s);
void launch_moddown_rescale_conv(const DeviceTables& t, const KsShape& sh, u64* conv, const u64* accP, const u64* top, const u64* hatinv,
                                 const u64* hatmod, const u64* mmod, hipStream_t s);
void launch_moddown_rescale_finish(const DeviceTables& t, const KsShape& sh, u64* out, const u64* accQ, const u64* conv, const u64* minv,
                                   hipStream_t s);
struct AffineItems {
    static constexpr int MAX_ITEMS = 32;
    const u64* add[MAX_ITEMS] = {};
    u32 f2 = 0, neg = 0, cst = 0;
};
void launch_affine_acc_items(const DeviceTables& t, const KsShape& sh, const AffineItems& it, u64* accQ, u64* accP, const u64* d,
                             const u64* consts, const u64* pmod, hipStream_t s);
void launch_moddown_rescale_exact_conv(const DeviceTables& t, const KsShape& sh, u32 f2, u64* conv, const u64* accP, const u64* phatinv,
                                       const u64* phatmod, const u64* pinv, const u64* pmod, const u64* qlm, hipStream_t s);
void launch_moddown_finish(const DeviceTables& t, const KsShape& sh, u64* out, const u64* accQ, const u64* conv, const u64* pinv,
                           const u64* add0, const u64* add1, const u32* map, const u64* post, hipStream_t s);

}
```

### fhe-linformer_amd/csrc/kernels_ks.hip

```cpp
#include <hip/hip_runtime.h>
#include <cstdlib>
#include "kernels.h"
#include "kernels_elem.h"

namespace fhelin {
namespace {

typedef u64 u64x2 __attribute__((ext_vector_type(2)));

__device__ __forceinline__ Barrett load_barrett(const DeviceTables& t, int limb) {
    Barrett b;
    b.q = t.moduli[limb];
    b.r0 = t.barrett[2 * limb];
    b.r1 = t.barrett[2 * limb + 1];
    return b;
}

constexpr int TCH = 16;

template <int MAXA, bool FULL>
__device__ __forceinline__ void modup_body(const DeviceTables& t, const KsShape& sh, u64* __restrict__ ext, const u64* __restrict__ cc,
                                           const u64* __restrict__ hatinv, const u64* __restrict__ hatmod, int j, int lo, int cnt, size_t n) {
    const size_t N = (size_t)1 << t.log_n;
    const int nt = sh.ell + sh.k;
// ... 547 lines not shown
        r.y = mul_shoup(sub_mod(a.y, b.y, q), w, ws, q);
        if (add) {
            const u64x2 d = reinterpret_cast<const u64x2*>(add)[((size_t)tt * N + j) >> 1];
            r.x = add_mod(r.x, d.x, q);
            r.y = add_mod(r.y, d.y, q);
        }
    }
    if (post) {
        const u64x2 p = reinterpret_cast<const u64x2*>(post)[((size_t)v * N + j) >> 1];
        r.x = add_mod(r.x, p.x, q);
        r.y = add_mod(r.y, p.y, q);
    }
    if (sh.gsrc && !sh.gsrc_pmod && c == 0) {
        const u64* __restrict__ g = sh.gsrc + (size_t)bi * sh.gsrc_stride + (size_t)tt * N;
        for (int rr = 0; rr < sh.n_rot; ++rr) {
            const u64* __restrict__ gr = g + (size_t)rr * sh.rot_input_stride;
            const u32* __restrict__ mr = sh.map_rot[rr];
            const u32 m0 = mr ? mr[j] : (u32)j;
            const u64x2 gp = reinterpret_cast<const u64x2*>(gr)[m0 >> 1];
            r.x = add_mod(r.x, (m0 & 1) ? gp.y : gp.x, q);
            r.y = add_mod(r.y, (m0 & 1) ? gp.x : gp.y, q);
        }
    }
    reinterpret_cast<u64x2*>(out)[((size_t)v * N + j) >> 1] = r;
}

__global__ __launch_bounds__(256) void fold_key_kernel(DeviceTables t, u64* __restrict__ out, const u64* __restrict__ key, const u32* __restrict__ map,
                                                       const u64* __restrict__ V) {
    const size_t v = blockIdx.y;
    const int limb = (int)(v % (size_t)t.n_limbs);
    const Barrett br = load_barrett(t, limb);
    const size_t N = (size_t)1 << t.log_n;
    const size_t j = ((size_t)blockIdx.x * 256 + threadIdx.x) * 2;
    const u32 m0 = map[j], m1 = map[j + 1];
    const u64x2 pv = reinterpret_cast<const u64x2*>(V)[((size_t)limb * N + j) >> 1];
    u64x2 r;
    const u64 R = t.mont[2 * limb], Rs = t.mont[2 * limb + 1];
    r.x = pack30(mul_shoup(mul_mod(pv.x, key[v * N + m0], br), R, Rs, br.q));
    r.y = pack30(mul_shoup(mul_mod(pv.y, key[v * N + m1], br), R, Rs, br.q));
    reinterpret_cast<u64x2*>(out)[(v * N + j) >> 1] = r;
}

__global__ __launch_bounds__(256) void hoist_addends_kernel(DeviceTables t, KsShape sh, HoistAdd h, u64* __restrict__ pre, const u64* __restrict__ ct) {
    const int bi = blockIdx.y / (2 * sh.ell), v = blockIdx.y % (2 * sh.ell);
    const int c = v / sh.ell, tt = v % sh.ell;
    const Barrett br = load_barrett(t, tt);
    const size_t N = (size_t)1 << t.log_n, row = N >> 1;
    const size_t n2 = (size_t)blockIdx.x * 256 + threadIdx.x;
    const u64x2* __restrict__ src = reinterpret_cast<const u64x2*>(ct + (size_t)bi * sh.c_stride + (size_t)v * N);
    const u64x2 x = src[n2];
    const u64x2 p0 = reinterpret_cast<const u64x2*>(h.v[0])[(size_t)tt * row + n2];
    Acc128 a0 = {0, 0}, a1 = {0, 0};
    acc_mac(a0, x.x, p0.x);
    acc_mac(a1, x.y, p0.y);
    if (c == 0)
        for (int r = 0; r < h.n_rot; ++r) {
            const u32 m0 = h.map[r][2 * n2];
            const u64x2 g = src[m0 >> 1];
            const u64x2 pr = reinterpret_cast<const u64x2*>(h.v[r + 1])[(size_t)tt * row + n2];
            acc_mac(a0, (m0 & 1) ? g.y : g.x, pr.x);
            acc_mac(a1, (m0 & 1) ? g.x : g.y, pr.y);
        }
    u64x2 o;
    o.x = barrett_reduce128(a0.lo, a0.hi, br);
    o.y = barrett_reduce128(a1.lo, a1.hi, br);
    if (h.acc) {
        u64x2* A = reinterpret_cast<u64x2*>(h.acc + (size_t)bi * 2 * sh.ell * N) + (size_t)v * row + n2;
        const u64 w = h.pmod[2 * tt], ws = h.pmod[2 * tt + 1];
        u64x2 a = *A;
        a.x = add_mod(a.x, mul_shoup(o.x, w, ws, br.q), br.q);
        a.y = add_mod(a.y, mul_shoup(o.y, w, ws, br.q), br.q);
        *A = a;
        return;
    }
    reinterpret_cast<u64x2*>(pre + (size_t)bi * 2 * sh.ell * N)[(size_t)v * row + n2] = o;
}

__global__ __launch_bounds__(256) void affine_acc_kernel(DeviceTables t, KsShape sh, u64* __restrict__ accQ, const u64* __restrict__ d,
                                                         const u64* __restrict__ sub, ScalarSet cst, int has_cst, int f, const u64* __restrict__ pmod) {
    const int bi = blockIdx.y / (2 * sh.ell), v = blockIdx.y % (2 * sh.ell);
    const int c = v / sh.ell, tt = v % sh.ell;
    const u64 q = t.moduli[tt];
    const size_t row = ((size_t)1 << t.log_n) >> 1;
    const size_t n2 = (size_t)blockIdx.x * 256 + threadIdx.x;
    u64x2 x = reinterpret_cast<const u64x2*>(d)[((size_t)bi * 3 * sh.ell + v) * row + n2];
    if (f == 2) {
        x.x = add_mod(x.x, x.x, q);
        x.y = add_mod(x.y, x.y, q);
    }
    if (has_cst && c == 0) {
        x.x = add_mod(x.x, cst.v[2 * tt], q);
        x.y = add_mod(x.y, cst.v[2 * tt], q);
    }
    if (sub) {
        const u64x2 sv = reinterpret_cast<const u64x2*>(sub)[((size_t)bi * 2 * sh.ell + v) * row + n2];
        x.x = sub_mod(x.x, sv.x, q);
        x.y = sub_mod(x.y, sv.y, q);
    }
    u64x2* A = reinterpret_cast<u64x2*>(accQ) + ((size_t)bi * 2 * sh.ell + v) * row + n2;
    u64x2 a = *A;
    if (f == 2) {
        a.x = add_mod(a.x, a.x, q);
        a.y = add_mod(a.y, a.y, q);
    }
    const u64 w = pmod[2 * tt], ws = pmod[2 * tt + 1];
    a.x = add_mod(a.x, mul_shoup(x.x, w, ws, q), q);
    a.y = add_mod(a.y, mul_shoup(x.y, w, ws, q), q);
    *A = a;
}

__global__ __launch_bounds__(256) void moddown_rescale_conv_kernel(DeviceTables t, KsShape sh, u64* __restrict__ conv, const u64* __restrict__ accP,
                                                                   const u64* __restrict__ top, const u64* __restrict__ hatinv,
                                                                   const u64* __restrict__ hatmod, const u64* __restrict__ mmod) {
    constexpr int MAXS = 16;
    const int bi = blockIdx.y >> 1, c = blockIdx.y & 1;
    const size_t N = (size_t)1 << t.log_n;
    const size_t n = (size_t)blockIdx.x * 256 + threadIdx.x;
    const int e1 = sh.ell - 1, ns = sh.k + 1;
    u32 z0[MAXS], z1[MAXS];
    u32 neg = 0;
#pragma unroll
    for (int p = 0; p < MAXS; ++p) {
        if (p < ns) {
            const u64 x = p < sh.k ? accP[(((size_t)bi * 2 + c) * sh.k + p) * N + n] : top[((size_t)bi * 2 + c) * N + n];
            const u64 m = t.moduli[p < sh.k ? sh.L1 + p : sh.ell - 1];
            const u64 y = mul_shoup(x, hatinv[2 * p], hatinv[2 * p + 1], m);
            neg += y > (m >> 1);
            split30(y, z0[p], z1[p]);
        } else {
            z0[p] = z1[p] = 0;
        }
    }
    u64* dst = conv + ((size_t)bi * 2 + c) * e1 * N + n;
    const int t0 = blockIdx.z * sh.tch, t1 = min(e1, t0 + sh.tch);
    for (int tt = t0; tt < t1; ++tt) {
        const Barrett br = load_barrett(t, tt);
        u64 slo = 0, shi = 0;
#pragma unroll
        for (int p0 = 0; p0 < MAXS; p0 += 8) {
            Acc30 acc = {0, 0, 0};
#pragma unroll
            for (int p = p0; p < p0 + 8; ++p)
                if (p < ns) {
                    const u64 hm = hatmod[(size_t)p * e1 + tt];
                    mac30(acc, z0[p], z1[p], (u32)hm, (u32)(hm >> 32));
                }
            acc30_flush(acc, slo, shi);
        }
        dst[(size_t)tt * N] = sub_mod(barrett_reduce128(slo, shi, br), barrett_reduce128((u64)neg * mmod[tt], 0, br), br.q);
    }
}

__global__ __launch_bounds__(256) void affine_acc_items_kernel(DeviceTables t, KsShape sh, AffineItems it, u64* __restrict__ accQ, u64* __restrict__ accP,
                                                               const u64* __restrict__ d, const u64* __restrict__ consts, const u64* __restrict__ pmod) {
    const int bi = blockIdx.y / (2 * sh.ell), v = blockIdx.y % (2 * sh.ell);
    const int c = v / sh.ell, tt = v % sh.ell;
    const bool f2 = (it.f2 >> bi) & 1;
    const size_t row = ((size_t)1 << t.log_n) >> 1;
    const size_t n2 = (size_t)blockIdx.x * 256 + threadIdx.x;
    const u64 q = t.moduli[tt];
    u64x2 x = reinterpret_cast<const u64x2*>(d)[(((size_t)bi * 3 + c) * sh.ell + tt) * row + n2];
    if (f2) {
        x.x = add_mod(x.x, x.x, q);
        x.y = add_mod(x.y, x.y, q);
    }
    if (c == 0 && ((it.cst >> bi) & 1)) {
        const u64 k = consts[(size_t)bi * sh.ell + tt];
        x.x = add_mod(x.x, k, q);
        x.y = add_mod(x.y, k, q);
    }
    const u64* __restrict__ add = it.add[bi];
    if (add) {
        const u64x2 sv = reinterpret_cast<const u64x2*>(add)[((size_t)c * sh.ell + tt) * row + n2];
        if ((it.neg >> bi) & 1) {
            x.x = sub_mod(x.x, sv.x, q);
            x.y = sub_mod(x.y, sv.y, q);
        } else {
            x.x = add_mod(x.x, sv.x, q);
            x.y = add_mod(x.y, sv.y, q);
        }
    }
    u64x2* A = reinterpret_cast<u64x2*>(accQ) + (((size_t)bi * 2 + c) * sh.ell + tt) * row + n2;
    u64x2 a = *A;
    if (f2) {
        a.x = add_mod(a.x, a.x, q);
        a.y = add_mod(a.y, a.y, q);
    }
    const u64 w = pmod[2 * tt], ws = pmod[2 * tt + 1];
    a.x = add_mod(a.x, mul_shoup(x.x, w, ws, q), q);
    a.y = add_mod(a.y, mul_shoup(x.y, w, ws, q), q);
    if (tt == sh.ell - 1)
        reinterpret_cast<u64x2*>(accP)[(((size_t)bi * 2 + c) * (sh.k + 1) + sh.k) * row + n2] = a;
    else
        *A = a;
}

template <int MAXK, bool FULL>
__device__ __forceinline__ void moddown_exact_body(const DeviceTables& t, const KsShape& sh, bool f2, u64* __restrict__ dst, const u64* __restrict__ src,
                                                   const u64* __restrict__ phatinv, const u64* __restrict__ phatmod, const u64* __restrict__ pinv,
                                                   const u64* __restrict__ pmod, const u64* __restrict__ qlm) {
    const size_t N = (size_t)1 << t.log_n;
    u32 z0[MAXK], z1[MAXK];
#pragma unroll
    for (int p = 0; p < MAXK; ++p) {
        if (FULL || p < sh.k) {
            split30(mul_shoup(src[(size_t)p * N], phatinv[2 * p], phatinv[2 * p + 1], t.moduli[sh.L1 + p]), z0[p], z1[p]);
        } else {
            z0[p] = z1[p] = 0;
        }
    }
    auto conv_to = [&](int tt, u64 qt) {
        const u64 qti = t.qinv[tt];
        u64 slo = 0, shi = 0;
#pragma unroll
        for (int p0 = 0; p0 < MAXK; p0 += 8) {
            Acc30 acc = {0, 0, 0};
#pragma unroll
            for (int p = p0; p < p0 + 8 && p < MAXK; ++p)
                if (FULL || p < sh.k) {
                    const u64 h = phatmod[(size_t)p * sh.L1 + tt];
                    mac30(acc, z0[p], z1[p], (u32)h, (u32)(h >> 32));
                }
            acc30_flush(acc, slo, shi);
        }
        const u64 r = redc128(slo, shi, qt, qti);
        return f2 ? add_mod(r, r, qt) : r;
    };
    const int top = sh.ell - 1;
    const u64 qtop = t.moduli[top];
    const u64 xt = mul_shoup(sub_mod(src[(size_t)sh.k * N], conv_to(top, qtop), qtop), pinv[2 * top], pinv[2 * top + 1], qtop);
    const bool high = xt > (qtop >> 1);
    const int t0 = blockIdx.z * sh.tch, t1 = min(top, t0 + sh.tch);
    for (int tt = t0; tt < t1; ++tt) {
        const Barrett br = load_barrett(t, tt);
        u64 lift = barrett_reduce128(xt, 0, br);
        if (high) lift = sub_mod(lift, qlm[tt], br.q);
        dst[(size_t)tt * N] = add_mod(conv_to(tt, br.q), mul_shoup(lift, pmod[2 * tt], pmod[2 * tt + 1], br.q), br.q);
    }
}

template <int MAXK>
__global__ __launch_bounds__(256) void moddown_rescale_exact_conv_kernel(DeviceTables t, KsShape sh, u32 f2_mask, u64* __restrict__ conv,
                                                                         const u64* __restrict__ accP, const u64* __restrict__ phatinv,
                                                                         const u64* __restrict__ phatmod, const u64* __restrict__ pinv,
                                                                         const u64* __restrict__ pmod, const u64* __restrict__ qlm) {
    const int bi = blockIdx.y >> 1;
    const size_t N = (size_t)1 << t.log_n;
    const size_t n = (size_t)blockIdx.x * 256 + threadIdx.x;
    const bool f2 = (f2_mask >> bi) & 1;
    const u64* src = accP + (size_t)blockIdx.y * (sh.k + 1) * N + n;
    u64* dst = conv + (size_t)blockIdx.y * (sh.ell - 1) * N + n;
    if (sh.k == MAXK)
        moddown_exact_body<MAXK, true>(t, sh, f2, dst, src, phatinv, phatmod, pinv, pmod, qlm);
    else
        moddown_exact_body<MAXK, false>(t, sh, f2, dst, src, phatinv, phatmod, pinv, pmod, qlm);
}

__global__ __launch_bounds__(256) void moddown_rescale_finish_kernel(DeviceTables t, KsShape sh, u64* __restrict__ out, const u64* __restrict__ accQ,
                                                                     const u64* __restrict__ conv, const u64* __restrict__ minv) {
    const int e1 = sh.ell - 1;
    const int bi = blockIdx.y / (2 * e1), v = blockIdx.y % (2 * e1);
    const int c = v / e1, tt = v % e1;
    const u64 q = t.moduli[tt];
    const u64 w = minv[2 * tt], ws = minv[2 * tt + 1];
    const size_t row = ((size_t)1 << t.log_n) >> 1;
    const size_t n2 = (size_t)blockIdx.x * 256 + threadIdx.x;
    const u64x2 a = reinterpret_cast<const u64x2*>(accQ)[(((size_t)bi * 2 + c) * sh.ell + tt) * row + n2];
    const u64x2 b = reinterpret_cast<const u64x2*>(conv)[(((size_t)bi * 2 + c) * e1 + tt) * row + n2];
    u64x2 r;
    r.x = mul_shoup(sub_mod(a.x, b.x, q), w, ws, q);
    r.y = mul_shoup(sub_mod(a.y, b.y, q), w, ws, q);
    reinterpret_cast<u64x2*>(out + (size_t)bi * sh.out_stride)[(size_t)v * row + n2] = r;
}

}

void launch_fold_key(const DeviceTables& t, u64* out, const u64* key, const u32* map, const u64* V, int nvec, hipStream_t s) {
    hipLaunchKernelGGL(fold_key_kernel, dim3((1u << t.log_n) / 512, (unsigned)nvec), dim3(256), 0, s, t, out, key, map, V);
}
void launch_hoist_addends(const DeviceTables& t, const KsShape& sh, const HoistAdd& h, u64* pre, const u64* ct, hipStream_t s) {
    hipLaunchKernelGGL(hoist_addends_kernel, dim3((1u << t.log_n) / 512, (unsigned)(sh.batch * 2 * sh.ell)), dim3(256), 0, s, t, sh, h, pre, ct);
}

void launch_affine_acc(const DeviceTables& t, const KsShape& sh, u64* accQ, const u64* d, const u64* sub, const ScalarSet& cst, int has_cst, int f,
                       const u64* pmod, hipStream_t s) {
    hipLaunchKernelGGL(affine_acc_kernel, dim3((1u << t.log_n) / 512, (unsigned)(sh.batch * 2 * sh.ell)), dim3(256), 0, s, t, sh, accQ, d, sub, cst,
                       has_cst, f, pmod);
}
static int conv_tch(unsigned planes, int targets) {
    static const int force = [] {
        const char* e = std::getenv("FHELIN_CONV_CHUNKS");
        return e ? std::atoi(e) : 0;
    }();
    if (force || planes < 2048u) return TCH;
    return targets > TCH ? targets : TCH;
}
void launch_moddown_rescale_conv(const DeviceTables& t, const KsShape& sh_in, u64* conv, const u64* accP, const u64* top, const u64* hatinv,
                                 const u64* hatmod, const u64* mmod, hipStream_t s) {
    KsShape sh = sh_in;
    const unsigned nx = (1u << t.log_n) / 256;
    sh.tch = conv_tch(nx * (unsigned)(sh.batch * 2), sh.ell - 1);
    dim3 g(nx, (unsigned)(sh.batch * 2), (unsigned)((sh.ell - 1 + sh.tch - 1) / sh.tch));
    hipLaunchKernelGGL(moddown_rescale_conv_kernel, g, dim3(256), 0, s, t, sh, conv, accP, top, hatinv, hatmod, mmod);
}
void launch_affine_acc_items(const DeviceTables& t, const KsShape& sh, const AffineItems& it, u64* accQ, u64* accP, const u64* d,
                             const u64* consts, const u64* pmod, hipStream_t s) {
    dim3 g((1u << t.log_n) / 512, (unsigned)(sh.batch * 2 * sh.ell));
    hipLaunchKernelGGL(affine_acc_items_kernel, g, dim3(256), 0, s, t, sh, it, accQ, accP, d, consts, pmod);
}
void launch_moddown_rescale_exact_conv(const DeviceTables& t, const KsShape& sh_in, u32 f2, u64* conv, const u64* accP, const u64* phatinv,
                                       const u64* phatmod, const u64* pinv, const u64* pmod, const u64* qlm, hipStream_t s) {
    KsShape sh = sh_in;
    const unsigned nx = (1u << t.log_n) / 256;
    sh.tch = conv_tch(nx * (unsigned)(sh.batch * 2), sh.ell - 1);
    dim3 g(nx, (unsigned)(sh.batch * 2), (unsigned)((sh.ell - 1 + sh.tch - 1) / sh.tch));
#define FHELIN_MDX_CASE(K) case K: hipLaunchKernelGGL((moddown_rescale_exact_conv_kernel<K>), g, dim3(256), 0, s, t, sh, f2, conv, accP, phatinv, phatmod, pinv, pmod, qlm); break;
    switch (sh.k) {
        FHELIN_MDX_CASE(1) FHELIN_MDX_CASE(2) FHELIN_MDX_CASE(3) FHELIN_MDX_CASE(4)
        FHELIN_MDX_CASE(5) FHELIN_MDX_CASE(6) FHELIN_MDX_CASE(7) FHELIN_MDX_CASE(8)
        default: hipLaunchKernelGGL((moddown_rescale_exact_conv_kernel<16>), g, dim3(256), 0, s, t, sh, f2, conv, accP, phatinv, phatmod, pinv, pmod, qlm); break;
    }
#undef FHELIN_MDX_CASE
}
void launch_moddown_rescale_finish(const DeviceTables& t, const KsShape& sh, u64* out, const u64* accQ, const u64* conv, const u64* minv,
                                   hipStream_t s) {
    dim3 g((1u << t.log_n) / 512, (unsigned)(sh.batch * 2 * (sh.ell - 1)));
    hipLaunchKernelGGL(moddown_rescale_finish_kernel, g, dim3(256), 0, s, t, sh, out, accQ, conv, minv);
}

void launch_modup_conv(const DeviceTables& t, const KsShape& sh_in, u64* ext, const u64* cc, const u64* c_ntt, const u64* hatinv,
                       const u64* hatmod, hipStream_t s) {
    KsShape sh = sh_in;
    const unsigned nx = (1u << t.log_n) / 256;
    sh.tch = conv_tch(nx * (unsigned)(sh.batch * sh.beta), sh.ell + sh.k);
    dim3 g(nx, (unsigned)(sh.batch * sh.beta), (unsigned)((sh.ell + sh.k + sh.tch - 1) / sh.tch));
#define FHELIN_MODUP_CASE(A) case A: hipLaunchKernelGGL((modup_conv_kernel<A>), g, dim3(256), 0, s, t, sh, ext, cc, c_ntt, hatinv, hatmod); break;
    switch (sh.alpha) {
        FHELIN_MODUP_CASE(1) FHELIN_MODUP_CASE(2) FHELIN_MODUP_CASE(3) FHELIN_MODUP_CASE(4)
        FHELIN_MODUP_CASE(5) FHELIN_MODUP_CASE(6) FHELIN_MODUP_CASE(7) FHELIN_MODUP_CASE(8)
        default: hipLaunchKernelGGL((modup_conv_kernel<16>), g, dim3(256), 0, s, t, sh, ext, cc, c_ntt, hatinv, hatmod); break;
    }
#undef FHELIN_MODUP_CASE
}
void launch_ks_inner(const DeviceTables& t, const KsShape& sh, u64* accQ, u64* accP, const u64* ext, const u64* evk, const u64* c_ntt,
                     hipStream_t s) {
    dim3 g((1u << t.log_n) / 512, (unsigned)(sh.batch * (sh.accp_rows ? sh.ell : sh.ell + sh.k)));
    if (sh.gather)
        hipLaunchKernelGGL(ks_inner_kernel<true>, g, dim3(256), 0, s, t, sh, accQ, accP, ext, evk, c_ntt);
    else
        hipLaunchKernelGGL(ks_inner_kernel<false>, g, dim3(256), 0, s, t, sh, accQ, accP, ext, evk, c_ntt);
}
void launch_ks_inner_multi(const DeviceTables& t, const KsShape& sh, u64* accQ, u64* accP, const u64* ext, const u64* c_ntt,
                           hipStream_t s) {
    static const int pair_rows = [] { const char* e = std::getenv("FHELIN_KS_ROW_PAIRS"); return e ? std::atoi(e) : 1; }();
    const bool stage = sh.lds_digits && sh.rot_ext_stride == 0 && sh.beta <= 4;
    const int nt = sh.accp_rows ? sh.ell : sh.ell + sh.k;
    if (pair_rows && sh.batch >= 2) {
        dim3 g((1u << t.log_n) / 512, (unsigned)(((sh.batch + 1) / 2) * nt));
        if (stage)
            hipLaunchKernelGGL((ks_inner_multi_kernel<true, 2>), g, dim3(256), 0, s, t, sh, accQ, accP, ext, c_ntt);
        else
            hipLaunchKernelGGL((ks_inner_multi_kernel<false, 2>), g, dim3(256), 0, s, t, sh, accQ, accP, ext, c_ntt);
        return;
    }
    dim3 g((1u << t.log_n) / 512, (unsigned)(sh.batch * nt));
    if (stage)
        hipLaunchKernelGGL((ks_inner_multi_kernel<true, 1>), g, dim3(256), 0, s, t, sh, accQ, accP, ext, c_ntt);
    else
        hipLaunchKernelGGL((ks_inner_multi_kernel<false, 1>), g, dim3(256), 0, s, t, sh, accQ, accP, ext, c_ntt);
}
void launch_ks_inner_dot(const DeviceTables& t, const KsShape& sh, const LtDot& ld, u64* accQ, u64* accP, const u64* ext, const u64* c0,
                         const u64* c1, hipStream_t s) {
    dim3 g((1u << t.log_n) / 512, (unsigned)(sh.batch * (sh.ell + sh.k)));
    if (ld.n_groups == 1)
        hipLaunchKernelGGL(ks_inner_dot_kernel<1>, g, dim3(256), 0, s, t, sh, ld, accQ, accP, ext, c0, c1);
    else if (ld.n_groups == 2)
        hipLaunchKernelGGL(ks_inner_dot_kernel<2>, g, dim3(256), 0, s, t, sh, ld, accQ, accP, ext, c0, c1);
    else
        hipLaunchKernelGGL((ks_inner_dot_kernel<LtStep::MAX_G>), g, dim3(256), 0, s, t, sh, ld, accQ, accP, ext, c0, c1);
}
void launch_moddown_conv(const DeviceTables& t, const KsShape& sh_in, u64* conv, const u64* accP, const u64* phatinv, const u64* phatmod,
                         hipStream_t s) {
    KsShape sh = sh_in;
    const unsigned nx = (1u << t.log_n) / 256;
    sh.tch = conv_tch(nx * (unsigned)(2 * sh.batch), sh.ell);
    dim3 g(nx, (unsigned)(2 * sh.batch), (unsigned)((sh.ell + sh.tch - 1) / sh.tch));
#define FHELIN_MODDOWN_CASE(K, S) case K: hipLaunchKernelGGL((moddown_conv_kernel<K, S>), g, dim3(256), 0, s, t, sh, conv, accP, phatinv, phatmod); break;
#define FHELIN_MODDOWN_SWITCH(S)                                                                                                                \
    switch (sh.k) {                                                                                                                             \
        FHELIN_MODDOWN_CASE(1, S) FHELIN_MODDOWN_CASE(2, S) FHELIN_MODDOWN_CASE(3, S) FHELIN_MODDOWN_CASE(4, S)                                 \
        FHELIN_MODDOWN_CASE(5, S) FHELIN_MODDOWN_CASE(6, S) FHELIN_MODDOWN_CASE(7, S) FHELIN_MODDOWN_CASE(8, S)                                 \
        default: hipLaunchKernelGGL((moddown_conv_kernel<16, S>), g, dim3(256), 0, s, t, sh, conv, accP, phatinv, phatmod); break;              \
    }
    if (sh.gather) {
        FHELIN_MODDOWN_SWITCH(true)
    } else {
        FHELIN_MODDOWN_SWITCH(false)
    }
#undef FHELIN_MODDOWN_SWITCH
#undef FHELIN_MODDOWN_CASE
}
void launch_moddown_finish(const DeviceTables& t, const KsShape& sh, u64* out, const u64* accQ, const u64* conv, const u64* pinv,
                           const u64* add0, const u64* add1, const u32* map, const u64* post, hipStream_t s) {
    dim3 g((1u << t.log_n) / 512, (unsigned)(sh.batch * 2 * sh.ell));
    hipLaunchKernelGGL(moddown_finish_kernel, g, dim3(256), 0, s, t, sh, out, accQ, conv, pinv, add0, add1, map, post);
}

}
```

### fhe-linformer_amd/csrc/kernels_ntt.hip

```cpp
#include <hip/hip_runtime.h>
#include <algorithm>
#include <cstdlib>
#include "kernels.h"
#include "kernels_elem.h"

namespace fhelin {

namespace {

struct NttArgs {
    u64* data;
    const u64* src;
    const u64* tw;
    const u64* tw_rows;
    const u64* moduli;
    const u64* ninv;
    const int* limb_tab;
    int tab_len;
    int limb_first;
    int limb_count;
    int log_n;
    int nvec;
    int period;
    int lazy_out;
// ... 290 lines not shown
        cols_body<A, INVERSE, true, LIFT>(a, lds, vec, tile, limb, c);
    else
        cols_body<A, INVERSE, false, LIFT>(a, lds, vec, tile, limb, c);
}

struct ProdOperands {
    const u64* ext;
    const u64* key0;
    const u32* map0;
    int n_rot;
    int khi;
    int tt, limb, comp;
    Barrett br;
    u64 qi;
    int own;
    const u64* own_src;
    u64 mont, monts;
    bool own_mont;
    const u64* gsrc;
    u64 pw, pws;
};
__device__ __forceinline__ void product_row(ProdOperands& o, const NttArgs& a, const NttProduct& pr, int bi, int& in) {
    const KsShape& sh = pr.sh;
    const size_t N = (size_t)1 << a.log_n;
    const int nt = sh.ell + sh.k;
    o.ext = pr.ext;
    o.key0 = pr.evk;
    o.map0 = nullptr;
    o.n_rot = 1;
    in = bi;
    if (pr.multi) {
        o.ext += (size_t)bi * (sh.ext_batch_stride ? sh.ext_batch_stride : (size_t)sh.beta * nt * N);
        o.n_rot = sh.n_rot;
    } else {
        int ri = 0;
        if (sh.row_mod) {
            ri = bi % sh.row_mod;
            in = bi / sh.row_mod;
            o.ext += (size_t)in * sh.ext_batch_stride;
            o.key0 = sh.evk_row[ri];
        } else {
            if (!sh.shared_input) o.ext += (size_t)bi * sh.beta * nt * N;
            if (sh.per_row) {
                ri = bi;
                o.key0 = sh.evk_row[bi];
            }
        }
        if (sh.gather) o.map0 = sh.map_row[ri];
    }
    o.khi = pr.multi || sh.gather ? 32 : 30;
}
__device__ __forceinline__ void product_limb(ProdOperands& o, int tt, int limb, int comp, u64 q, const u64* __restrict__ barrett,
                                             const u64* __restrict__ qinv) {
    o.tt = tt;
    o.limb = limb;
    o.comp = comp;
    o.br.q = q;
    o.br.r0 = barrett[2 * limb];
    o.br.r1 = barrett[2 * limb + 1];
    o.qi = qinv[limb];
}

template <int PG>
__device__ __forceinline__ void product_offsets(u32 (&off)[PG], const u32* map, int tile, int g, int tau) {
    if (map) {
        const Stream ms = stream(map + ((size_t)tile << 12));
#pragma unroll
        for (int i = 0; i < PG; ++i) off[i] = 8u * ld32(ms, 4u * (u32)tau, 1024 * i, 1024 * g);
    } else {
#pragma unroll
        for (int i = 0; i < PG; ++i) off[i] = ((u32)tile << 15) + 8u * (u32)tau + 2048u * (u32)(g + i);
    }
}

template <int PG, bool SHORT, bool OWN>
__device__ __forceinline__ void product_sums(u64 (&res)[PG], const NttArgs& a, const NttProduct& pr, const ProdOperands& o, int tile, int g,
                                             int tau) {
    const KsShape& sh = pr.sh;
    const int log_n = a.log_n;
    const int nt = sh.ell + sh.k;
    const size_t kstride = (size_t)(sh.L1 + sh.k) << log_n;
    const size_t klimb = ((size_t)o.limb << log_n) + ((size_t)tile << 12);
    const u32 lane8 = 8u * (u32)tau;
    u64 lo[PG], hi[PG];
    Acc30 acc[PG];
#pragma unroll
    for (int i = 0; i < PG; ++i) {
        lo[i] = hi[i] = 0;
        acc[i] = Acc30{0, 0, 0};
    }
    int pending = 0, folded = 0;
#pragma unroll 1
    for (int r = 0; r < o.n_rot; ++r) {
        const u32* map = pr.multi ? sh.map_rot[r] : o.map0;
        const u64* key = pr.multi ? sh.evk_rot[r] : o.key0;
        const u64* dig = o.ext + (size_t)r * sh.rot_ext_stride + ((size_t)o.tt << log_n);
        u32 off[PG];
        product_offsets<PG>(off, map, tile, g, tau);
#pragma unroll 1
        for (int j = 0; j < sh.beta; ++j) {
            const bool is_own = OWN && j == o.own;
            const Stream ds = stream(is_own ? o.own_src : dig + ((size_t)j * nt << log_n));
            const Stream ks = stream(key + (size_t)(2 * j + o.comp) * kstride + klimb);
            u64 d[PG], kw[PG];
#pragma unroll
            for (int i = 0; i < PG; ++i) {
                d[i] = ld64(ds, off[i], 0);
                kw[i] = ld64(ks, lane8, 2048 * i, 2048 * g);
            }
            if constexpr (OWN) {
                if (is_own && o.own_mont) {
#pragma unroll
                    for (int i = 0; i < PG; ++i) d[i] = mul_shoup(d[i], o.mont, o.monts, o.br.q);
                }
            }
#pragma unroll
            for (int i = 0; i < PG; ++i) {
                u32 d0, d1;
                split30(d[i], d0, d1);
                mac30(acc[i], d0, d1, (u32)kw[i] & 0x3FFFFFFFu, (u32)(kw[i] >> o.khi));
            }
            if (!SHORT && ++pending == 8) {
                pending = 0;
                const bool fold = ++folded == 2;
                if (fold) folded = 0;
#pragma unroll
                for (int i = 0; i < PG; ++i) {
                    acc30_flush(acc[i], lo[i], hi[i]);
                    acc[i] = Acc30{0, 0, 0};
                    if (fold) {
                        lo[i] = barrett_reduce128(lo[i], hi[i], o.br);
                        hi[i] = 0;
                    }
                }
            }
        }
    }
#pragma unroll
    for (int i = 0; i < PG; ++i) {
        acc30_flush(acc[i], lo[i], hi[i]);
        res[i] = redc128(lo[i], hi[i], o.br.q, o.qi);
    }
    if constexpr (OWN) {
        if (o.gsrc) {
            u32 off[PG];
            product_offsets<PG>(off, o.map0, tile, g, tau);
            const Stream gs = stream(o.gsrc);
#pragma unroll
            for (int i = 0; i < PG; ++i) res[i] = add_mod(res[i], mul_shoup(ld64(gs, off[i], 0), o.pw, o.pws, o.br.q), o.br.q);
        }
    }
}

template <int PG, bool SHORT>
__device__ __forceinline__ void product_to_lds(u64* lds, const NttArgs& a, const NttProduct& pr, const u64* __restrict__ barrett,
                                               const u64* __restrict__ qinv, int vec, int tile, int limb, u64 q, int tau) {
    const KsShape& sh = pr.sh;
    const int K = sh.k;
    const int poly = uniform(vec / K), p = vec - poly * K;
    ProdOperands o;
    int in;
    product_row(o, a, pr, poly >> 1, in);
    product_limb(o, sh.ell + p, limb, poly & 1, q, barrett, qinv);
    u64* const from = lds + lds_slot(tile_index(tau, 0, 8));
#pragma unroll 1
    for (int g = 0; g < 16; g += PG) {
        u64 res[PG];
        product_sums<PG, SHORT, false>(res, a, pr, o, tile, g, tau);
        u64* const fg = from + lds_slot(tile_index(0, 1, 8)) * g;
#pragma unroll
        for (int i = 0; i < PG; ++i) fg[lds_slot(tile_index(0, i, 8))] = res[i];
    }
}

template <int NK>
__device__ __forceinline__ void epilogue_finish(u64 (&x)[NK], const u64 (&av)[NK], int g, const NttEpilogue* ep, const LimbConst& c, u64 epi_b,
                                                int log_n, int tile, int tau, int poly, int t, int ell) {
    const u32 lane8 = 8u * (u32)tile_index(tau, 0, 8);
    auto koff = [](int k) constexpr { return 8 * tile_index(0, k, 8); };
    const int goff = koff(1) * g;
    const int bi = poly >> 1, comp = poly & 1;
    const size_t n = (size_t)1 << log_n;
    const u64 w = ep->w[2 * t], ws = ep->w[2 * t + 1];
#pragma unroll
    for (int k = 0; k < NK; ++k) x[k] = mul_shoup(av[k] + epi_b - x[k], w, ws, c.q);
    const u64* add = comp == 0 ? ep->add0 : ep->add1;
    if (add) {
        const Stream adds = stream(add + (size_t)bi * ep->add_stride + (size_t)t * n + ((size_t)tile << 12));
#pragma unroll
        for (int k = 0; k < NK; ++k) x[k] = add_mod(x[k], ld64(adds, lane8, koff(k), goff), c.q);
    }
    const size_t row_off = (size_t)(comp * ell + t) * n;
    const bool has_post = ep->post != nullptr;
    const Stream post = stream(ep->post + (has_post ? (size_t)bi * ep->post_stride + row_off : 0));
    const Stream out = stream(ep->out + (size_t)bi * ep->out_stride + row_off);
    const int toff = (tile << 15) + goff;
    const u32* im = ep->per_row ? ep->invmap_row[bi] : ep->invmap;
    if (im) {
        const Stream ims = stream(im + ((size_t)tile << 12));
#pragma unroll
        for (int k = 0; k < NK; ++k) {
            const u32 j8 = 8u * ld32(ims, 4u * (u32)tau, 4 * tile_index(0, k, 8), goff >> 1);
            u64 r = x[k];
            if (has_post) r = add_mod(r, ld64(post, j8, 0), c.q);
            st64(out, j8, 0, r);
        }
    } else {
        if (has_post) {
#pragma unroll
            for (int k = 0; k < NK; ++k) x[k] = add_mod(x[k], ld64(post, lane8, koff(k), toff), c.q);
        }
#pragma unroll
        for (int k = 0; k < NK; ++k) st64(out, lane8, koff(k), x[k], toff);
    }
}

struct ProdTabs {
    const NttProduct* pr;
    const u64* barrett;
    const u64* qinv;
    const u64* mont;
};

template <int PG, bool SHORT>
__device__ __forceinline__ void epilogue_products(const u64* lds, const NttArgs& a, const NttEpilogue* ep, const ProdTabs& pt, const LimbConst& c,
                                                  u64 epi_b, bool reduce_x, int tile, int tau, int poly, int t, int ell) {
    const NttProduct& pr = *pt.pr;
    const KsShape& sh = pr.sh;
    const int log_n = a.log_n;
    const int bi = poly >> 1, comp = poly & 1;
    ProdOperands o;
    int in;
    product_row(o, a, pr, bi, in);
    product_limb(o, t, t, comp, c.q, pt.barrett, pt.qinv);
    o.own = t / sh.alpha;
    const int cin = sh.row_mod ? in : sh.shared_input ? 0 : bi;
    o.own_src = pr.c_ntt + (size_t)cin * sh.c_stride + ((size_t)t << log_n);
    o.own_mont = !sh.gather;
    o.mont = pt.mont[2 * t];
    o.monts = pt.mont[2 * t + 1];
    o.gsrc = nullptr;
    o.pw = o.pws = 0;
    if (sh.gather && sh.gsrc_pmod && comp == 0) {
        o.gsrc = sh.gsrc + (size_t)in * sh.gsrc_stride + ((size_t)t << log_n);
        o.pw = sh.gsrc_pmod[2 * t];
        o.pws = sh.gsrc_pmod[2 * t + 1];
    }
    const u64* const to = lds + lds_slot(tile_index(tau, 0, 8));
#pragma unroll 1
    for (int g = 0; g < 16; g += PG) {
        u64 av[PG], x[PG];
        product_sums<PG, SHORT, true>(av, a, pr, o, tile, g, tau);
        const u64* const tg = to + lds_slot(tile_index(0, 1, 8)) * g;
#pragma unroll
        for (int i = 0; i < PG; ++i) x[i] = tg[lds_slot(tile_index(0, i, 8))];
        if (reduce_x) {
#pragma unroll
            for (int i = 0; i < PG; ++i) x[i] = reduce_lazy_2q(x[i], c.q, c.sh, c.rr);
        }
        epilogue_finish<PG>(x, av, g, ep, c, epi_b, log_n, tile, tau, poly, t, ell);
    }
}

template <bool INVERSE, bool LAZY, bool EPI, bool PROD = false>
__device__ __forceinline__ void rows_body(const NttArgs& a, u64* lds, int vec, int tile, int limb, const LimbConst& c,
                                          const NttEpilogue* ep, const ProdTabs* pt = nullptr) {
    const int log_n = a.log_n;
    const Stream tw = stream(reinterpret_cast<const u64x2*>(a.tw) + ((size_t)limb << log_n));
    const Stream trows = stream(reinterpret_cast<const u64x2*>(a.tw_rows) + (((size_t)limb << (log_n - 12)) + tile) * (15 * 256));
    [[maybe_unused]] u64* const vbase = a.data + ((size_t)vec << log_n) + ((size_t)tile << 12);
    const Stream base = stream(vbase);
    const Stream sbase = stream(a.src + src_offset(a, vec, log_n) + ((size_t)tile << 12));
    const int tau = threadIdx.x;
    const u32 lane4 = 8u * (u32)tile_index(tau, 0, 4), lane8 = 8u * (u32)tile_index(tau, 0, 8);
    auto koff = [](int k, int p) constexpr { return 8 * tile_index(0, k, p); };
    u64 x[16];

    if (!INVERSE) {
#pragma unroll
        for (int k = 0; k < 16; ++k) x[k] = ld64(sbase, lane4, koff(k, 4));
        RoundTw rt, rn;
        load_round_tw<0, 4>(rt, tw, log_n, 4, tile << 4, tau >> 4);
        fwd_round<0, 4, LAZY>(x, rt, c);
        load_round_tw_rows(rn, trows, tau);
        exchange(x, lds, tau, 4, 0, false);
        fwd_round<0, 4, LAZY>(x, rn, c);
        [[maybe_unused]] u64 av[16];
        [[maybe_unused]] int ell = 0, t = 0, poly = 0;
        if constexpr (EPI) {
            ell = ep->ell;
            poly = uniform(vec / ell);
            t = vec - poly * ell;
        }
        if constexpr (EPI && !PROD) {
            const Stream acc = stream(ep->acc + (size_t)poly * ep->acc_poly_stride + ((size_t)t << log_n) + ((size_t)tile << 12));
#pragma unroll
            for (int k = 0; k < 16; ++k) av[k] = ld64(acc, lane8, koff(k, 8));
        }
        [[maybe_unused]] u64 epi_b = 0;
        if constexpr (EPI) {
            if (LAZY) {
                epi_b = 86 * c.q;
            } else if (c.q < (1ull << 60)) {
                epi_b = 10 * c.q;
            } else {
                epi_b = 2 * c.q;
                if constexpr (!PROD) {
#pragma unroll
                    for (int k = 0; k < 16; ++k) x[k] = reduce_lazy_2q(x[k], c.q, c.sh, c.rr);
                }
            }
        } else if (!(LAZY && a.lazy_out && c.q < (1ull << 53))) {
#pragma unroll
            for (int k = 0; k < 16; ++k)
                x[k] = csub_mask(reduce_lazy_2q(x[k], c.q, c.sh, c.rr), c.q);
        }
#if defined(FHELIN_ROWS_DIRECT_STORE)
        if constexpr (!EPI) {
#pragma unroll
            for (int k = 0; k < 16; k += 2) {
                u64x2 v;
                v.x = x[k];
                v.y = x[k + 1];
                reinterpret_cast<u64x2*>(vbase + 16 * tau)[k >> 1] = v;
            }
            return;
        }
#endif
        if constexpr (EPI && PROD) {
            park(x, lds, tau, 0, true);
            const bool reduce_x = !LAZY && c.q >= (1ull << 60);
            if (pt->pr->sh.beta <= 8)
                epilogue_products<8, true>(lds, a, ep, *pt, c, epi_b, reduce_x, tile, tau, poly, t, ell);
            else
                epilogue_products<4, false>(lds, a, ep, *pt, c, epi_b, reduce_x, tile, tau, poly, t, ell);
        } else {
            exchange(x, lds, tau, 0, 8, true);
            if constexpr (EPI) {
                epilogue_finish<16>(x, av, 0, ep, c, epi_b, log_n, tile, tau, poly, t, ell);
            } else {
#pragma unroll
                for (int k = 0; k < 16; ++k) st64(base, lane8, koff(k, 8), x[k]);
            }
        }
    } else {
        RoundTw rt, rn;
        if constexpr (PROD) {
            load_round_tw_rows(rt, trows, tau);
            __syncthreads();
            const u64* const to = lds + lds_slot(tile_index(tau, 0, 0));
#pragma unroll
            for (int k = 0; k < 16; ++k) x[k] = to[lds_slot(tile_index(0, k, 0))];
        } else {
#pragma unroll
            for (int k = 0; k < 16; ++k) x[k] = ld64(sbase, lane8, koff(k, 8));
            load_round_tw_rows(rt, trows, tau);
            exchange(x, lds, tau, 8, 0, false);
        }
        inv_round<0, 4, false, LAZY, 0, 1>(x, rt, c, nullptr);
        load_round_tw<0, 4>(rn, tw, log_n, 4, tile << 4, tau >> 4);
        exchange(x, lds, tau, 0, 4, true);
        inv_round<0, 4, false, LAZY, 4, 1>(x, rn, c, nullptr);
        if (LAZY) {
#pragma unroll
            for (int k = 0; k < 16; ++k) x[k] = reduce_lazy_2q(x[k], c.q, c.sh, c.rr);
        }
#pragma unroll
        for (int k = 0; k < 16; ++k) st64(base, lane4, koff(k, 4), x[k]);
    }
}

__device__ __forceinline__ void rows_block(const NttArgs& a, int& vec, int& tile) {
    const int logtiles = a.log_n - 12;
    int lid = blockIdx.x;
    const int nblk = gridDim.x;
    if ((nblk & 7) == 0) lid = (lid & 7) * (nblk >> 3) + (lid >> 3);
    if (a.period > 0) {
        const int nper = a.nvec / a.period;
        const int rep = lid % nper, r = lid / nper;
        tile = r & ((1 << logtiles) - 1);
        vec = a.vec0 + rep * a.period + (r >> logtiles);
    } else {
        vec = a.vec0 + (lid >> logtiles);
        tile = lid & ((1 << logtiles) - 1);
    }
    vec = uniform(vec);
    tile = uniform(tile);
}

template <bool INVERSE, bool EPI = false>
__global__ __launch_bounds__(256) __attribute__((amdgpu_waves_per_eu(4))) void ntt_rows_kernel(NttArgs a, NttEpilogue ep) {
    __shared__ u64 lds[LDS_WORDS];
    int vec, tile;
    rows_block(a, vec, tile);
    const int limb = uniform(limb_of(a, vec));
    if (limb < 0) return;
    const LimbConst c = limb_const(a, limb);
    if (lazy_prime<INVERSE>(c.q))
        rows_body<INVERSE, true, EPI>(a, lds, vec, tile, limb, c, &ep);
    else
        rows_body<INVERSE, false, EPI>(a, lds, vec, tile, limb, c, &ep);
}

__global__ __launch_bounds__(256) __attribute__((amdgpu_waves_per_eu(4))) void ntt_rows_product_kernel(NttArgs a, NttProduct pr, const u64* barrett,
                                                                                                        const u64* qinv) {
    __shared__ u64 lds[LDS_WORDS];
    int vec, tile;
    rows_block(a, vec, tile);
    const int limb = uniform(limb_of(a, vec));
    const LimbConst c = limb_const(a, limb);
    if ((pr.multi ? pr.sh.n_rot : 1) * pr.sh.beta <= 8)
        product_to_lds<8, true>(lds, a, pr, barrett, qinv, vec, tile, limb, c.q, threadIdx.x);
    else
        product_to_lds<4, false>(lds, a, pr, barrett, qinv, vec, tile, limb, c.q, threadIdx.x);
    if (lazy_prime<true>(c.q))
        rows_body<true, true, false, true>(a, lds, vec, tile, limb, c, nullptr);
    else
        rows_body<true, false, false, true>(a, lds, vec, tile, limb, c, nullptr);
}

__global__ __launch_bounds__(256) __attribute__((amdgpu_waves_per_eu(4))) void ntt_rows_epilogue_product_kernel(NttArgs a, NttEpilogue ep, NttProduct pr,
                                                                                                                 const u64* barrett, const u64* qinv,
                                                                                                                 const u64* mont) {
    __shared__ u64 lds[LDS_WORDS];
    int vec, tile;
    rows_block(a, vec, tile);
    const int limb = uniform(limb_of(a, vec));
    const LimbConst c = limb_const(a, limb);
    const ProdTabs pt{&pr, barrett, qinv, mont};
    if (lazy_prime<false>(c.q))
        rows_body<false, true, true, true>(a, lds, vec, tile, limb, c, &ep, &pt);
    else
        rows_body<false, false, true, true>(a, lds, vec, tile, limb, c, &ep, &pt);
}

template <int A>
void launch_cols(const NttArgs& a, bool inverse, int blocks, hipStream_t s) {
    if (inverse)
        hipLaunchKernelGGL((ntt_cols_kernel<A, true>), dim3(blocks), dim3(256), 0, s, a);
    else if (a.lift_qlm)
        hipLaunchKernelGGL((ntt_cols_kernel<A, false, true>), dim3(blocks), dim3(256), 0, s, a);
    else
        hipLaunchKernelGGL((ntt_cols_kernel<A, false>), dim3(blocks), dim3(256), 0, s, a);
}

}

enum NttPasses { BOTH_PASSES, ROWS_PRODUCT, COLS_ONLY };
static void launch_ntt_impl(const DeviceTables& t, const LimbBatch& b, bool inverse, const NttEpilogue* ep, hipStream_t s,
                            NttPasses which = BOTH_PASSES, const NttProduct* prod = nullptr);

void launch_ntt(const DeviceTables& t, const LimbBatch& b, bool inverse, hipStream_t s) { launch_ntt_impl(t, b, inverse, nullptr, s); }
void launch_ntt_epilogue(const DeviceTables& t, const LimbBatch& b, const NttEpilogue& ep, hipStream_t s) {
    launch_ntt_impl(t, b, false, &ep, s);
}
void launch_ntt_rows_product(const DeviceTables& t, const LimbBatch& b, const NttProduct& p, hipStream_t s) {
    launch_ntt_impl(t, b, true, nullptr, s, ROWS_PRODUCT, &p);
}
void launch_ntt_cols_inverse(const DeviceTables& t, const LimbBatch& b, hipStream_t s) { launch_ntt_impl(t, b, true, nullptr, s, COLS_ONLY); }
void launch_ntt_epilogue_product(const DeviceTables& t, const LimbBatch& b, const NttEpilogue& ep, const NttProduct& p, hipStream_t s) {
    launch_ntt_impl(t, b, false, &ep, s, BOTH_PASSES, &p);
}

static void launch_ntt_impl(const DeviceTables& t, const LimbBatch& b, bool inverse, const NttEpilogue* ep, hipStream_t s, NttPasses which,
                            const NttProduct* prod) {
    if (b.nvec <= 0) return;
    NttArgs a;
    a.data = b.data;
    a.src = b.src ? b.src : b.data;
    a.src_group = b.src ? b.src_group : 0;
    a.src_group_stride = b.src_group_stride;
    a.src_group2 = (b.src && b.src_group > 0) ? b.src_group2 : 0;
    a.src_group2_stride = b.src_group2_stride;
    a.lazy_out = (!inverse && b.lazy_out) ? 1 : 0;
    a.lift_qlm = (!inverse && b.src && b.lift_limb >= 0) ? b.lift_qlm : nullptr;
    a.lift_limb = b.lift_limb;
    a.tw = inverse ? t.tw_inv : t.tw_fwd;
    a.tw_rows = inverse ? t.tw_rows_inv : t.tw_rows_fwd;
    a.moduli = t.moduli;
    a.ninv = t.ninv;
    a.limb_tab = b.limb_tab;
    a.tab_len = b.tab_len;
    a.limb_first = b.limb_first;
    a.limb_count = b.limb_count > 0 ? b.limb_count : 1;
    a.log_n = t.log_n;
    a.nvec = b.nvec;
    const int per = b.limb_tab ? b.tab_len : a.limb_count;
    a.period = (per > 0 && per < b.nvec && b.nvec % per == 0) ? per : 0;
    const int A = t.log_n - 8;
    a.vec0 = 0;
    static const int chunk_mb = [] {
        const char* e = std::getenv("FHELIN_NTT_CHUNK_MB");
        return e ? std::atoi(e) : 0;
    }();
    int chunk = b.nvec;
    if (chunk_mb > 0 && !ep && which == BOTH_PASSES) {
        const size_t vec_bytes = (size_t)8 << t.log_n;
        const int want = (int)std::max<size_t>(1, ((size_t)chunk_mb << 20) / vec_bytes);
        if (b.nvec > want + want / 2) {
            const int per = a.period > 0 ? a.period : 1;
            chunk = std::max(per, want / per * per);
        }
    }
    const int nvec_all = b.nvec, period_all = a.period;
    const u64* src_all = a.src;
    const int sg = a.src_group, sg2 = a.src_group2;
    for (int v0 = 0; v0 < nvec_all; v0 += chunk) {
        a.vec0 = v0;
        a.nvec = std::min(chunk, nvec_all - v0);
        a.period = (period_all > 0 && a.nvec % period_all == 0 && a.nvec > period_all) ? period_all : 0;
        a.src = src_all;
        a.src_group = sg;
        a.src_group2 = sg2;
        const int blocks = a.nvec << (t.log_n - 12);
        auto cols = [&]() {
            switch (A) {
                case 4: launch_cols<4>(a, inverse, blocks, s); break;
                case 5: launch_cols<5>(a, inverse, blocks, s); break;
                case 6: launch_cols<6>(a, inverse, blocks, s); break;
                case 7: launch_cols<7>(a, inverse, blocks, s); break;
                case 8: launch_cols<8>(a, inverse, blocks, s); break;
                case 9: launch_cols<9>(a, inverse, blocks, s); break;
                default: break;
            }
        };
        if (!inverse) {
            cols();
            a.src = a.data;
            a.src_group = 0;
            a.src_group2 = 0;
            if (ep && prod)
                hipLaunchKernelGGL(ntt_rows_epilogue_product_kernel, dim3(blocks), dim3(256), 0, s, a, *ep, *prod, t.barrett, t.qinv, t.mont);
            else if (ep)
                hipLaunchKernelGGL((ntt_rows_kernel<false, true>), dim3(blocks), dim3(256), 0, s, a, *ep);
            else
                hipLaunchKernelGGL((ntt_rows_kernel<false, false>), dim3(blocks), dim3(256), 0, s, a, NttEpilogue());
        } else {
            if (which == ROWS_PRODUCT) {
                hipLaunchKernelGGL(ntt_rows_product_kernel, dim3(blocks), dim3(256), 0, s, a, *prod, t.barrett, t.qinv);
                continue;
            }
            if (which != COLS_ONLY) hipLaunchKernelGGL((ntt_rows_kernel<true, false>), dim3(blocks), dim3(256), 0, s, a, NttEpilogue());
            a.src = a.data;
            a.src_group = 0;
            a.src_group2 = 0;
            cols();
        }
    }
}

}
```

Baseline: 217.7.

## Fuse affine accumulation of exact keyswitch tail into NTT row passes; cache affine constants

```diff
diff --git a/fhe-linformer_amd/csrc/context.cpp b/fhe-linformer_amd/csrc/context.cpp
--- a/fhe-linformer_amd/csrc/context.cpp
+++ b/fhe-linformer_amd/csrc/context.cpp
@@ -129,6 +129,7 @@
         if (const char* e = std::getenv("FHELIN_ACCP_ROWS_MIN_VECS")) accp_rows_min_vecs = std::atoi(e);
         if (const char* e = std::getenv("FHELIN_FUSE_ACCQ_ROWS")) fuse_accq_rows = std::atoi(e);
         if (const char* e = std::getenv("FHELIN_ACCQ_ROWS_MIN_VECS")) accq_rows_min_vecs = std::atoi(e);
+        if (const char* e = std::getenv("FHELIN_FUSE_EXACT_ROWS")) fuse_exact_rows = std::atoi(e);
         if (const char* e = std::getenv("FHELIN_NTT_TRACE")) trace_small_ntt = std::atoi(e);
         if (const char* e = std::getenv("FHELIN_SCALAR_TRACE")) trace_scalar = std::atoi(e);
         if (const char* e = std::getenv("FHELIN_HOST_WAITS")) trace_waits = std::atoi(e) != 0;
diff --git a/fhe-linformer_amd/csrc/context.h b/fhe-linformer_amd/csrc/context.h
--- a/fhe-linformer_amd/csrc/context.h
+++ b/fhe-linformer_amd/csrc/context.h
@@ -170,6 +170,7 @@
     int accp_rows_min_vecs = 0;
     int fuse_accq_rows = 1;
     int accq_rows_min_vecs = 0;
+    int fuse_exact_rows = 0;
     bool lds_digits = true;
     struct FftDev {
         const u32* rot = nullptr;
@@ -200,10 +201,10 @@
         if (trace_small_ntt && b.nvec <= trace_small_ntt) note_small_ntt(b.nvec);
         launch_ntt_epilogue(dt, b, ep, stream);
     }
-    void ntt_epilogue_product(const LimbBatch& b, const NttEpilogue& ep, const NttProduct& p) {
+    void ntt_epilogue_product(const LimbBatch& b, const NttEpilogue& ep, const NttProduct& p, const NttAffine* af = nullptr) {
         stats.limb_ntt += (u64)b.nvec;
         if (trace_small_ntt && b.nvec <= trace_small_ntt) note_small_ntt(b.nvec);
-        launch_ntt_epilogue_product(dt, b, ep, p, stream);
+        launch_ntt_epilogue_product(dt, b, ep, p, stream, af);
     }
 };
 
diff --git a/fhe-linformer_amd/csrc/evaluator.cpp b/fhe-linformer_amd/csrc/evaluator.cpp
--- a/fhe-linformer_amd/csrc/evaluator.cpp
+++ b/fhe-linformer_amd/csrc/evaluator.cpp
@@ -1,4 +1,5 @@
 #include "evaluator.h"
+#include <algorithm>
 #include <map>
 #include <set>
 #include <hip/hip_runtime.h>
@@ -305,15 +306,42 @@
     return tail == KsTail::RowPass && !sh.n_rot && want;
 }
 
+bool Evaluator::exact_in_rows(const KsShape& sh, KsTail tail) const {
+    const bool measured_faster = sh.beta <= 8;
+    const bool want = c_.fuse_exact_rows >= 2 || (c_.fuse_exact_rows == 1 && measured_faster);
+    return tail == KsTail::Exact && want && c_.fuse_accp_rows && c_.fuse_accq_rows && c_.fuse_finish && !sh.n_rot && sh.k == c_.K &&
+           sh.accp_limbs == c_.K + 1;
+}
+
 Evaluator::KsAcc Evaluator::accumulators(const KsShape& sh, KsTail tail) {
     const size_t pairs = (size_t)sh.batch * 2 * c_.N;
     return KsAcc{sh, tail, c_.scratch<u64>(pairs * sh.ell), c_.scratch<u64>(pairs * (sh.accp_limbs ? sh.accp_limbs : sh.k)), {}};
 }
 
-Evaluator::KsAcc Evaluator::inner_product(const KsShape& shape, const u64* ext, const u64* evk, const u64* c_ntt, KsTail tail) {
+Evaluator::KsAcc Evaluator::inner_product(const KsShape& shape, const u64* ext, const u64* evk, const u64* c_ntt, KsTail tail,
+                                          const NttAffine* aff) {
     const int K = c_.K, nvec = shape.batch * 2 * K;
     KsAcc acc{shape, tail, {}, {}, {}};
     KsShape& sh = acc.sh;
+    if (tail == KsTail::Exact) {
+        if (!aff || sh.accp_limbs != K + 1 || sh.n_rot) throw Error(FHELIN_ERR_INTERNAL, "inner_product: the exact tail's shape");
+        const int nvx = sh.batch * 2 * (K + 1);
+        sh.accp_rows = sh.accq_rows = exact_in_rows(sh, tail) ? 1 : 0;
+        acc.accP = c_.scratch<u64>((size_t)nvx * c_.N);
+        if (!sh.accq_rows) {
+            acc.accQ = c_.scratch<u64>((size_t)sh.batch * 2 * sh.ell * c_.N);
+            launch_ks_inner(c_.dt, sh, acc.accQ, acc.accP, ext, evk, c_ntt, c_.stream);
+            launch_affine_acc_items(c_.dt, sh, aff->it, acc.accQ, acc.accP, aff->d, aff->pmod, c_.stream);
+            return acc;
+        }
+        acc.qprod = NttProduct{sh, ext, evk, 0, c_ntt};
+        acc.aff = *aff;
+        c_.stats.limb_ntt += (u64)nvx;
+        LimbBatch ib{acc.accP, nvx, c_.lvl[sh.ell].mdx_limb_tab, 0, 1};
+        ib.tab_len = K + 1;
+        launch_ntt_rows_product(c_.dt, ib, acc.qprod, c_.stream, &acc.aff);
+        return acc;
+    }
     sh.accp_rows = accp_in_rows(sh, tail) ? 1 : 0;
     sh.accq_rows = sh.accp_rows && accq_in_rows(sh, tail) ? 1 : 0;
     if (!sh.accq_rows) acc.accQ = c_.scratch<u64>((size_t)sh.batch * 2 * sh.ell * c_.N);
@@ -408,7 +436,8 @@
     {
         LimbBatch ib{acc.accP, B * 2 * (K + 1), lt.mdx_limb_tab, 0, 1};
         ib.tab_len = K + 1;
-        c_.ntt(ib, true);
+        if (sh.accp_rows) launch_ntt_cols_inverse(c_.dt, ib, c_.stream);
+        else c_.ntt(ib, true);
     }
     Scratch<u64> conv = c_.scratch<u64>((size_t)B * 2 * (ell - 1) * c_.N);
     launch_moddown_rescale_exact_conv(c_.dt, sh, f2, conv, acc.accP, c_.d_phatinv, c_.d_phatmod, c_.d_pinv, c_.d_pmod,
@@ -428,9 +457,11 @@
         ep.out_stride = sh.out_stride;
         ep.w = minv;
         ep.ell = e1;
-        c_.ntt_epilogue(cb, ep);
+        if (sh.accq_rows) c_.ntt_epilogue_product(cb, ep, acc.qprod, &acc.aff);
+        else c_.ntt_epilogue(cb, ep);
         return;
     }
+    if (sh.accq_rows) throw Error(FHELIN_ERR_INTERNAL, "moddown_rescale_finish: the accumulator was left to a row pass that does not run");
     c_.ntt(cb, false);
     launch_moddown_rescale_finish(c_.dt, sh, out, acc.accQ, conv, minv, c_.stream);
 }
@@ -1747,6 +1778,51 @@
     return rescale_batch(t);
 }
 
+Evaluator::~Evaluator() {
+    for (AffineConst& e : affine_consts_) {
+        (void)hipEventDestroy(e.ready);
+        try {
+            c_.pool.free(e.d, e.lanes);
+        } catch (...) {
+        }
+    }
+}
+
+const u64* Evaluator::affine_const_row(double cadd, long double scale, int ell) {
+    const int lane = c_.pool.cur_lane;
+    for (AffineConst& e : affine_consts_)
+        if (e.cadd == cadd && e.scale == scale && e.ell == ell) {
+            if (!(e.lanes >> lane & 1)) {
+                if (lane != e.lane) hip_check(hipStreamWaitEvent(c_.stream, e.ready, 0), "hipStreamWaitEvent(affine constants)");
+                e.lanes |= 1u << lane;
+            }
+            std::rotate(&e, &e + 1, affine_consts_.data() + affine_consts_.size());
+            return affine_consts_.back().d;
+        }
+    if (affine_consts_.size() >= MAX_AFFINE_CONSTS) {
+        AffineConst& old = affine_consts_.front();
+        (void)hipEventDestroy(old.ready);
+        c_.pool.free(old.d, old.lanes);
+        affine_consts_.erase(affine_consts_.begin());
+    }
+    ScalarSet one;
+    real_to_scalars(c_, (long double)cadd * scale, ell, one);
+    std::vector<u64> row(ell);
+    for (int l = 0; l < ell; ++l) row[l] = one.v[2 * l];
+    AffineConst e{cadd, scale, ell, c_.dalloc<u64>((size_t)ell), lane, 1u << lane, nullptr};
+    try {
+        hip_check(hipEventCreateWithFlags(&e.ready, hipEventDisableTiming), "hipEventCreate(affine constants)");
+        c_.upload_async(e.d, row.data(), row.size());
+        hip_check(hipEventRecord(e.ready, c_.stream), "hipEventRecord(affine constants)");
+    } catch (...) {
+        if (e.ready) (void)hipEventDestroy(e.ready);
+        c_.pool.free(e.d);
+        throw;
+    }
+    affine_consts_.push_back(e);
+    return e.d;
+}
+
 std::vector<CtPtr> Evaluator::mult_affine_batch(const std::vector<CtPtr>& a, const std::vector<CtPtr>& b, const std::vector<AffineSpec>& spec) {
     if (a.size() != b.size() || spec.size() != a.size()) throw Error(FHELIN_ERR_ARG, "mult_affine_batch: operand count mismatch");
     if (!relin_key) throw Error(FHELIN_ERR_KEY, "no relinearisation key (EvalMultKeyGen not called)");
@@ -1763,7 +1839,6 @@
         if (x[i]->ell < 2 || (spec[i].addend && spec[i].addend->ell < x[i]->ell)) return mult_affine_unmerged(x, y, spec);
     const size_t N = c_.N;
     const int K = c_.K;
-    hipStream_t s = c_.stream;
     static_assert(AffineItems::MAX_ITEMS <= EwItems::MAX_ITEMS, "the tensor products of a group are one launch");
     return for_groups(n, std::min(batch_limit, (int)AffineItems::MAX_ITEMS), [&](size_t f, size_t i) { return x[i]->ell == x[f]->ell; },
                       [&](const std::vector<size_t>& idx) {
@@ -1774,7 +1849,6 @@
         AffineItems items;
         std::vector<CtPtr> adj(B);
         std::map<std::pair<const Ciphertext*, long double>, CtPtr> adjusted;
-        std::vector<u64> cst((size_t)B * ell, 0);
         for (int k = 0; k < B; ++k) {
             const size_t i = idx[k];
             const AffineSpec& sp = spec[i];
@@ -1793,15 +1867,8 @@
                 items.add[k] = adj[k]->d;
                 if (sp.negate) items.neg |= 1u << k;
             }
-            if (sp.cadd != 0.0) {
-                ScalarSet one;
-                real_to_scalars(c_, (long double)sp.cadd * sc, ell, one);
-                for (int l = 0; l < ell; ++l) cst[(size_t)k * ell + l] = one.v[2 * l];
-                items.cst |= 1u << k;
-            }
-        }
-        Scratch<u64> dcst = c_.scratch<u64>(cst.size());
-        if (items.cst) c_.upload_async(dcst, cst.data(), cst.size());
+            if (sp.cadd != 0.0) items.cst[k] = affine_const_row(sp.cadd, sc, ell);
+        }
         KsShape sh = ks_shape(ell, B, {3 * pn, (size_t)2 * (ell - 1) * N, pn});
         sh.accp_limbs = K + 1;
         c_.stats.keyswitch += (u64)B;
@@ -1812,9 +1879,8 @@
         std::vector<CtPtr> o = new_ct_batch(B, 2, ell - 1, 1, 0, x[first]->slots);
         {
             Scratch<u64> ext = modup(sh, c_ntt, true);
-            KsAcc acc = accumulators(sh, KsTail::Exact);
-            launch_ks_inner(c_.dt, sh, acc.accQ, acc.accP, ext, relin_key->d, c_ntt, s);
-            launch_affine_acc_items(c_.dt, sh, items, acc.accQ, acc.accP, d[0]->d, dcst, c_.d_pmod, s);
+            const NttAffine aff{items, d[0]->d, c_.d_pmod};
+            KsAcc acc = inner_product(sh, ext, relin_key->d, c_ntt, KsTail::Exact, &aff);
             moddown_rescale_exact(acc, o[0]->d, items.f2);
             launch_ok("mult_affine_batch");
         }
diff --git a/fhe-linformer_amd/csrc/evaluator.h b/fhe-linformer_amd/csrc/evaluator.h
--- a/fhe-linformer_amd/csrc/evaluator.h
+++ b/fhe-linformer_amd/csrc/evaluator.h
@@ -102,6 +102,9 @@
 class Evaluator {
 public:
     explicit Evaluator(Context& c) : c_(c) {}
+    ~Evaluator();
+    Evaluator(const Evaluator&) = delete;
+    Evaluator& operator=(const Evaluator&) = delete;
     Context& ctx() { return c_; }
 
     CtPtr new_ct(int npoly, int ell, int deg, long double scale, int slots);
@@ -240,6 +243,19 @@
 
 private:
     Context& c_;
+    struct AffineConst {
+        double cadd;
+        long double scale;
+        int ell;
+        u64* d;
+        int lane;
+        unsigned lanes;
+        hipEvent_t ready;
+    };
+    static constexpr size_t MAX_AFFINE_CONSTS = 64;
+    static_assert(MAX_AFFINE_CONSTS > AffineItems::MAX_ITEMS, "a call's rows are never the next to go");
+    std::vector<AffineConst> affine_consts_;
+    const u64* affine_const_row(double cadd, long double scale, int ell);
     void keyswitch_impl(int batch, const KsRows* rows, const u64* c_ntt, size_t c_stride, int ell, const EvalKey* key, u64* out,
                         size_t out_stride, const u64* add0, const u64* add1, size_t add_stride, const u32* map, const u64* post,
                         size_t post_stride);
@@ -258,6 +274,7 @@
         Scratch<u64> accQ;
         Scratch<u64> accP;
         NttProduct qprod;
+        NttAffine aff;
     };
     struct KsOut {
         u64* out = nullptr;
@@ -268,10 +285,11 @@
     KsTail moddown_tail(KsOutput o) const;
     const u64* set_gather(KsShape& sh, const EvalKey* const* keys, const u32* const* maps, const u64* c0 = nullptr, size_t c0_stride = 0);
     Scratch<u64> modup(const KsShape& up, const u64* src, bool times_r2, int group2 = 0, size_t group2_stride = 0);
-    KsAcc inner_product(const KsShape& sh, const u64* ext, const u64* evk, const u64* c_ntt, KsTail tail);
+    KsAcc inner_product(const KsShape& sh, const u64* ext, const u64* evk, const u64* c_ntt, KsTail tail, const NttAffine* aff = nullptr);
     KsAcc accumulators(const KsShape& sh, KsTail tail);
     bool accp_in_rows(const KsShape& sh, KsTail tail) const;
     bool accq_in_rows(const KsShape& sh, KsTail tail) const;
+    bool exact_in_rows(const KsShape& sh, KsTail tail) const;
     void accp_inverse(KsAcc& acc);
     Scratch<u64> moddown_conv(KsAcc& acc);
     void moddown(KsAcc& acc, const KsOut& o);
diff --git a/fhe-linformer_amd/csrc/kernels_elem.h b/fhe-linformer_amd/csrc/kernels_elem.h
--- a/fhe-linformer_amd/csrc/kernels_elem.h
+++ b/fhe-linformer_amd/csrc/kernels_elem.h
@@ -168,8 +168,10 @@
     int multi = 0;
     const u64* c_ntt = nullptr;
 };
-void launch_ntt_rows_product(const DeviceTables& t, const LimbBatch& b, const NttProduct& p, hipStream_t s);
-void launch_ntt_epilogue_product(const DeviceTables& t, const LimbBatch& b, const NttEpilogue& ep, const NttProduct& p, hipStream_t s);
+struct NttAffine;
+void launch_ntt_rows_product(const DeviceTables& t, const LimbBatch& b, const NttProduct& p, hipStream_t s, const NttAffine* af = nullptr);
+void launch_ntt_epilogue_product(const DeviceTables& t, const LimbBatch& b, const NttEpilogue& ep, const NttProduct& p, hipStream_t s,
+                                 const NttAffine* af = nullptr);
 void launch_ntt_cols_inverse(const DeviceTables& t, const LimbBatch& b, hipStream_t s);
 void launch_modup_conv(const DeviceTables& t, const KsShape& sh, u64* ext, const u64* cc, const u64* c_ntt, const u64* hatinv,
                        const u64* hatmod, hipStream_t s);
@@ -216,10 +218,16 @@
 struct AffineItems {
     static constexpr int MAX_ITEMS = 32;
     const u64* add[MAX_ITEMS] = {};
-    u32 f2 = 0, neg = 0, cst = 0;
+    const u64* cst[MAX_ITEMS] = {};
+    u32 f2 = 0, neg = 0;
+};
+struct NttAffine {
+    AffineItems it;
+    const u64* d = nullptr;
+    const u64* pmod = nullptr;
 };
 void launch_affine_acc_items(const DeviceTables& t, const KsShape& sh, const AffineItems& it, u64* accQ, u64* accP, const u64* d,
-                             const u64* consts, const u64* pmod, hipStream_t s);
+                             const u64* pmod, hipStream_t s);
 void launch_moddown_rescale_exact_conv(const DeviceTables& t, const KsShape& sh, u32 f2, u64* conv, const u64* accP, const u64* phatinv,
                                        const u64* phatmod, const u64* pinv, const u64* pmod, const u64* qlm, hipStream_t s);
 void launch_moddown_finish(const DeviceTables& t, const KsShape& sh, u64* out, const u64* accQ, const u64* conv, const u64* pinv,
diff --git a/fhe-linformer_amd/csrc/kernels_ks.hip b/fhe-linformer_amd/csrc/kernels_ks.hip
--- a/fhe-linformer_amd/csrc/kernels_ks.hip
+++ b/fhe-linformer_amd/csrc/kernels_ks.hip
@@ -723,7 +723,7 @@
 }
 
 __global__ __launch_bounds__(256) void affine_acc_items_kernel(DeviceTables t, KsShape sh, AffineItems it, u64* __restrict__ accQ, u64* __restrict__ accP,
-                                                               const u64* __restrict__ d, const u64* __restrict__ consts, const u64* __restrict__ pmod) {
+                                                               const u64* __restrict__ d, const u64* __restrict__ pmod) {
     const int bi = blockIdx.y / (2 * sh.ell), v = blockIdx.y % (2 * sh.ell);
     const int c = v / sh.ell, tt = v % sh.ell;
     const bool f2 = (it.f2 >> bi) & 1;
@@ -735,8 +735,8 @@
         x.x = add_mod(x.x, x.x, q);
         x.y = add_mod(x.y, x.y, q);
     }
-    if (c == 0 && ((it.cst >> bi) & 1)) {
-        const u64 k = consts[(size_t)bi * sh.ell + tt];
+    if (c == 0 && it.cst[bi]) {
+        const u64 k = it.cst[bi][tt];
         x.x = add_mod(x.x, k, q);
         x.y = add_mod(x.y, k, q);
     }
@@ -875,9 +875,9 @@
     hipLaunchKernelGGL(moddown_rescale_conv_kernel, g, dim3(256), 0, s, t, sh, conv, accP, top, hatinv, hatmod, mmod);
 }
 void launch_affine_acc_items(const DeviceTables& t, const KsShape& sh, const AffineItems& it, u64* accQ, u64* accP, const u64* d,
-                             const u64* consts, const u64* pmod, hipStream_t s) {
+                             const u64* pmod, hipStream_t s) {
     dim3 g((1u << t.log_n) / 512, (unsigned)(sh.batch * 2 * sh.ell));
-    hipLaunchKernelGGL(affine_acc_items_kernel, g, dim3(256), 0, s, t, sh, it, accQ, accP, d, consts, pmod);
+    hipLaunchKernelGGL(affine_acc_items_kernel, g, dim3(256), 0, s, t, sh, it, accQ, accP, d, pmod);
 }
 void launch_moddown_rescale_exact_conv(const DeviceTables& t, const KsShape& sh_in, u32 f2, u64* conv, const u64* accP, const u64* phatinv,
                                        const u64* phatmod, const u64* pinv, const u64* pmod, const u64* qlm, hipStream_t s) {
diff --git a/fhe-linformer_amd/csrc/kernels_ntt.hip b/fhe-linformer_amd/csrc/kernels_ntt.hip
--- a/fhe-linformer_amd/csrc/kernels_ntt.hip
+++ b/fhe-linformer_amd/csrc/kernels_ntt.hip
@@ -466,17 +466,90 @@
     }
 }
 
-template <int PG, bool SHORT>
+__device__ __forceinline__ void product_own(ProdOperands& o, const NttProduct& pr, const u64* __restrict__ mont, int bi, int in, int t, int log_n) {
+    const KsShape& sh = pr.sh;
+    o.own = t / sh.alpha;
+    const int cin = sh.row_mod ? in : sh.shared_input ? 0 : bi;
+    o.own_src = pr.c_ntt + (size_t)cin * sh.c_stride + ((size_t)t << log_n);
+    o.own_mont = !sh.gather;
+    o.mont = mont[2 * t];
+    o.monts = mont[2 * t + 1];
+    o.gsrc = nullptr;
+    o.pw = o.pws = 0;
+}
+
+template <int PG>
+__device__ __forceinline__ void affine_step(u64 (&S)[PG], const NttAffine& af, const KsShape& sh, int bi, int comp, int t, u64 q, int log_n, int tile,
+                                            int g, int tau) {
+    const u32 lane8 = 8u * (u32)tau;
+    const size_t pos = ((size_t)t << log_n) + ((size_t)tile << 12);
+    const bool f2 = (af.it.f2 >> bi) & 1;
+    const Stream ds = stream(af.d + (((size_t)bi * 3 + comp) * sh.ell << log_n) + pos);
+    u64 x[PG];
+#pragma unroll
+    for (int i = 0; i < PG; ++i) x[i] = ld64(ds, lane8, 2048 * i, 2048 * g);
+    if (f2) {
+#pragma unroll
+        for (int i = 0; i < PG; ++i) x[i] = add_mod(x[i], x[i], q);
+    }
+    const u64* cst = af.it.cst[bi];
+    if (comp == 0 && cst) {
+        const u64 k = cst[t];
+#pragma unroll
+        for (int i = 0; i < PG; ++i) x[i] = add_mod(x[i], k, q);
+    }
+    const u64* add = af.it.add[bi];
+    if (add) {
+        const Stream as = stream(add + ((size_t)comp * sh.ell << log_n) + pos);
+        u64 sv[PG];
+#pragma unroll
+        for (int i = 0; i < PG; ++i) sv[i] = ld64(as, lane8, 2048 * i, 2048 * g);
+        if ((af.it.neg >> bi) & 1) {
+#pragma unroll
+            for (int i = 0; i < PG; ++i) x[i] = sub_mod(x[i], sv[i], q);
+        } else {
+#pragma unroll
+            for (int i = 0; i < PG; ++i) x[i] = add_mod(x[i], sv[i], q);
+        }
+    }
+    if (f2) {
+#pragma unroll
+        for (int i = 0; i < PG; ++i) S[i] = add_mod(S[i], S[i], q);
+    }
+    const u64 w = af.pmod[2 * t], ws = af.pmod[2 * t + 1];
+#pragma unroll
+    for (int i = 0; i < PG; ++i) S[i] = add_mod(S[i], mul_shoup(x[i], w, ws, q), q);
+}
+
+template <int PG, bool SHORT, bool AFF = false>
 __device__ __forceinline__ void product_to_lds(u64* lds, const NttArgs& a, const NttProduct& pr, const u64* __restrict__ barrett,
-                                               const u64* __restrict__ qinv, int vec, int tile, int limb, u64 q, int tau) {
+                                               const u64* __restrict__ qinv, int vec, int tile, int limb, u64 q, int tau,
+                                               const NttAffine* af = nullptr, const u64* __restrict__ mont = nullptr) {
     const KsShape& sh = pr.sh;
-    const int K = sh.k;
+    const int K = AFF ? sh.k + 1 : sh.k;
     const int poly = uniform(vec / K), p = vec - poly * K;
     ProdOperands o;
     int in;
     product_row(o, a, pr, poly >> 1, in);
+    u64* const from = lds + lds_slot(tile_index(tau, 0, 8));
+    if constexpr (AFF) {
+        if (p == sh.k) {
+            const int top = sh.ell - 1;
+            product_limb(o, top, top, poly & 1, q, barrett, qinv);
+            product_own(o, pr, mont, poly >> 1, in, top, a.log_n);
+#pragma unroll 1
+            for (int g = 0; g < 16; g += PG) {
+                u64 res[PG];
+                product_sums<PG, SHORT, true>(res, a, pr, o, tile, g, tau);
+                affine_step<PG>(res, *af, sh, poly >> 1, poly & 1, top, q, a.log_n, tile, g, tau);
+                u64* const fg = from + lds_slot(tile_index(0, 1, 8)) * g;
+#pragma unroll
+                for (int i = 0; i < PG; ++i) fg[lds_slot(tile_index(0, i, 8))] = res[i];
+            }
+            return;
+        }
+    }
     product_limb(o, sh.ell + p, limb, poly & 1, q, barrett, qinv);
-    u64* const from = lds + lds_slot(tile_index(tau, 0, 8));
 #pragma unroll 1
     for (int g = 0; g < 16; g += PG) {
         u64 res[PG];
@@ -534,9 +607,10 @@
     const u64* barrett;
     const u64* qinv;
     const u64* mont;
+    const NttAffine* af = nullptr;
 };
 
-template <int PG, bool SHORT>
+template <int PG, bool SHORT, bool AFF = false>
 __device__ __forceinline__ void epilogue_products(const u64* lds, const NttArgs& a, const NttEpilogue* ep, const ProdTabs& pt, const LimbConst& c,
                                                   u64 epi_b, bool reduce_x, int tile, int tau, int poly, int t, int ell) {
     const NttProduct& pr = *pt.pr;
@@ -547,14 +621,7 @@
     int in;
     product_row(o, a, pr, bi, in);
     product_limb(o, t, t, comp, c.q, pt.barrett, pt.qinv);
-    o.own = t / sh.alpha;
-    const int cin = sh.row_mod ? in : sh.shared_input ? 0 : bi;
-    o.own_src = pr.c_ntt + (size_t)cin * sh.c_stride + ((size_t)t << log_n);
-    o.own_mont = !sh.gather;
-    o.mont = pt.mont[2 * t];
-    o.monts = pt.mont[2 * t + 1];
-    o.gsrc = nullptr;
-    o.pw = o.pws = 0;
+    product_own(o, pr, pt.mont, bi, in, t, log_n);
     if (sh.gather && sh.gsrc_pmod && comp == 0) {
         o.gsrc = sh.gsrc + (size_t)in * sh.gsrc_stride + ((size_t)t << log_n);
         o.pw = sh.gsrc_pmod[2 * t];
@@ -565,6 +632,7 @@
     for (int g = 0; g < 16; g += PG) {
         u64 av[PG], x[PG];
         product_sums<PG, SHORT, true>(av, a, pr, o, tile, g, tau);
+        if constexpr (AFF) affine_step<PG>(av, *pt.af, sh, bi, comp, t, c.q, log_n, tile, g, tau);
         const u64* const tg = to + lds_slot(tile_index(0, 1, 8)) * g;
 #pragma unroll
         for (int i = 0; i < PG; ++i) x[i] = tg[lds_slot(tile_index(0, i, 8))];
@@ -576,7 +644,7 @@
     }
 }
 
-template <bool INVERSE, bool LAZY, bool EPI, bool PROD = false>
+template <bool INVERSE, bool LAZY, bool EPI, bool PROD = false, bool AFF = false>
 __device__ __forceinline__ void rows_body(const NttArgs& a, u64* lds, int vec, int tile, int limb, const LimbConst& c,
                                           const NttEpilogue* ep, const ProdTabs* pt = nullptr) {
     const int log_n = a.log_n;
@@ -645,9 +713,9 @@
             park(x, lds, tau, 0, true);
             const bool reduce_x = !LAZY && c.q >= (1ull << 60);
             if (pt->pr->sh.beta <= 8)
-                epilogue_products<8, true>(lds, a, ep, *pt, c, epi_b, reduce_x, tile, tau, poly, t, ell);
+                epilogue_products<8, true, AFF>(lds, a, ep, *pt, c, epi_b, reduce_x, tile, tau, poly, t, ell);
             else
-                epilogue_products<4, false>(lds, a, ep, *pt, c, epi_b, reduce_x, tile, tau, poly, t, ell);
+                epilogue_products<4, false, AFF>(lds, a, ep, *pt, c, epi_b, reduce_x, tile, tau, poly, t, ell);
         } else {
             exchange(x, lds, tau, 0, 8, true);
             if constexpr (EPI) {
@@ -748,6 +816,38 @@
         rows_body<false, false, true, true>(a, lds, vec, tile, limb, c, &ep, &pt);
 }
 
+__global__ __launch_bounds__(256) __attribute__((amdgpu_waves_per_eu(4))) void ntt_rows_product_affine_kernel(NttArgs a, NttProduct pr, NttAffine af,
+                                                                                                               const u64* barrett, const u64* qinv,
+                                                                                                               const u64* mont) {
+    __shared__ u64 lds[LDS_WORDS];
+    int vec, tile;
+    rows_block(a, vec, tile);
+    const int limb = uniform(limb_of(a, vec));
+    const LimbConst c = limb_const(a, limb);
+    if (pr.sh.beta <= 8)
+        product_to_lds<8, true, true>(lds, a, pr, barrett, qinv, vec, tile, limb, c.q, threadIdx.x, &af, mont);
+    else
+        product_to_lds<4, false, true>(lds, a, pr, barrett, qinv, vec, tile, limb, c.q, threadIdx.x, &af, mont);
+    if (lazy_prime<true>(c.q))
+        rows_body<true, true, false, true>(a, lds, vec, tile, limb, c, nullptr);
+    else
+        rows_body<true, false, false, true>(a, lds, vec, tile, limb, c, nullptr);
+}
+__global__ __launch_bounds__(256) __attribute__((amdgpu_waves_per_eu(4))) void ntt_rows_epilogue_affine_kernel(NttArgs a, NttEpilogue ep, NttProduct pr,
+                                                                                                                NttAffine af, const u64* barrett,
+                                                                                                                const u64* qinv, const u64* mont) {
+    __shared__ u64 lds[LDS_WORDS];
+    int vec, tile;
+    rows_block(a, vec, tile);
+    const int limb = uniform(limb_of(a, vec));
+    const LimbConst c = limb_const(a, limb);
+    const ProdTabs pt{&pr, barrett, qinv, mont, &af};
+    if (lazy_prime<false>(c.q))
+        rows_body<false, true, true, true, true>(a, lds, vec, tile, limb, c, &ep, &pt);
+    else
+        rows_body<false, false, true, true, true>(a, lds, vec, tile, limb, c, &ep, &pt);
+}
+
 template <int A>
 void launch_cols(const NttArgs& a, bool inverse, int blocks, hipStream_t s) {
     if (inverse)
@@ -762,22 +862,23 @@
 
 enum NttPasses { BOTH_PASSES, ROWS_PRODUCT, COLS_ONLY };
 static void launch_ntt_impl(const DeviceTables& t, const LimbBatch& b, bool inverse, const NttEpilogue* ep, hipStream_t s,
-                            NttPasses which = BOTH_PASSES, const NttProduct* prod = nullptr);
+                            NttPasses which = BOTH_PASSES, const NttProduct* prod = nullptr, const NttAffine* af = nullptr);
 
 void launch_ntt(const DeviceTables& t, const LimbBatch& b, bool inverse, hipStream_t s) { launch_ntt_impl(t, b, inverse, nullptr, s); }
 void launch_ntt_epilogue(const DeviceTables& t, const LimbBatch& b, const NttEpilogue& ep, hipStream_t s) {
     launch_ntt_impl(t, b, false, &ep, s);
 }
-void launch_ntt_rows_product(const DeviceTables& t, const LimbBatch& b, const NttProduct& p, hipStream_t s) {
-    launch_ntt_impl(t, b, true, nullptr, s, ROWS_PRODUCT, &p);
+void launch_ntt_rows_product(const DeviceTables& t, const LimbBatch& b, const NttProduct& p, hipStream_t s, const NttAffine* af) {
+    launch_ntt_impl(t, b, true, nullptr, s, ROWS_PRODUCT, &p, af);
 }
 void launch_ntt_cols_inverse(const DeviceTables& t, const LimbBatch& b, hipStream_t s) { launch_ntt_impl(t, b, true, nullptr, s, COLS_ONLY); }
-void launch_ntt_epilogue_product(const DeviceTables& t, const LimbBatch& b, const NttEpilogue& ep, const NttProduct& p, hipStream_t s) {
-    launch_ntt_impl(t, b, false, &ep, s, BOTH_PASSES, &p);
+void launch_ntt_epilogue_product(const DeviceTables& t, const LimbBatch& b, const NttEpilogue& ep, const NttProduct& p, hipStream_t s,
+                                 const NttAffine* af) {
+    launch_ntt_impl(t, b, false, &ep, s, BOTH_PASSES, &p, af);
 }
 
 static void launch_ntt_impl(const DeviceTables& t, const LimbBatch& b, bool inverse, const NttEpilogue* ep, hipStream_t s, NttPasses which,
-                            const NttProduct* prod) {
+                            const NttProduct* prod, const NttAffine* af) {
     if (b.nvec <= 0) return;
     NttArgs a;
     a.data = b.data;
@@ -843,7 +944,9 @@
             a.src = a.data;
             a.src_group = 0;
             a.src_group2 = 0;
-            if (ep && prod)
+            if (ep && prod && af)
+                hipLaunchKernelGGL(ntt_rows_epilogue_affine_kernel, dim3(blocks), dim3(256), 0, s, a, *ep, *prod, *af, t.barrett, t.qinv, t.mont);
+            else if (ep && prod)
                 hipLaunchKernelGGL(ntt_rows_epilogue_product_kernel, dim3(blocks), dim3(256), 0, s, a, *ep, *prod, t.barrett, t.qinv, t.mont);
             else if (ep)
                 hipLaunchKernelGGL((ntt_rows_kernel<false, true>), dim3(blocks), dim3(256), 0, s, a, *ep);
@@ -851,7 +954,10 @@
                 hipLaunchKernelGGL((ntt_rows_kernel<false, false>), dim3(blocks), dim3(256), 0, s, a, NttEpilogue());
         } else {
             if (which == ROWS_PRODUCT) {
-                hipLaunchKernelGGL(ntt_rows_product_kernel, dim3(blocks), dim3(256), 0, s, a, *prod, t.barrett, t.qinv);
+                if (af)
+                    hipLaunchKernelGGL(ntt_rows_product_affine_kernel, dim3(blocks), dim3(256), 0, s, a, *prod, *af, t.barrett, t.qinv, t.mont);
+                else
+                    hipLaunchKernelGGL(ntt_rows_product_kernel, dim3(blocks), dim3(256), 0, s, a, *prod, t.barrett, t.qinv);
                 continue;
             }
             if (which != COLS_ONLY) hipLaunchKernelGGL((ntt_rows_kernel<true, false>), dim3(blocks), dim3(256), 0, s, a, NttEpilogue());
```

Measured after the change: 216.9, median of 5. About the same (-0.4%).
